# wpeebles/gangealing

Measured on NVIDIA H100. Metric: gangealing_train_images_per_sec_256, higher is better.
Workload: dtype f32

## Files before the change

gangealing_b200/_lib.py:

```python
import ctypes
import os

import torch

_HERE = os.path.dirname(os.path.abspath(__file__))
LIB_PATH = os.path.join(_HERE, "libgg_b200.so")

GG_F32, GG_F16, GG_BF16 = 0, 1, 2
PAD_MODES = {"zeros": 0, "border": 1, "reflection": 2}

_c = ctypes
_P, _I, _L, _F = _c.c_void_p, _c.c_int, _c.c_int64, _c.c_float

SIGNATURES = {
    "gg_version": (_I, []),
    "gg_last_error": (_c.c_char_p, []),
    "gg_sm_count": (_I, []),
    "gg_fused_bias_act": (_I, [_P, _P, _P, _P, _I, _I, _I, _F, _F, _L, _L, _L, _P]),
    "gg_noise_bias_act": (_I, [_P, _P, _P, _P, _P, _P, _I, _F, _F, _L, _L, _L, _P]),
    "gg_channel_scale_workspace": (_L, [_L, _L]),
    "gg_channel_scale": (_I, [_P, _P, _P, _P, _P, _P, _I, _L, _L, _P]),
    "gg_bias_act_backward_workspace": (_L, [_L, _L, _L]),
    "gg_bias_act_backward": (_I, [_P, _P, _P, _P, _P, _I, _F, _F, _L, _L, _L, _P]),
    "gg_upfirdn2d": (_I, [_P, _P, _P, _I, _L] + [_I] * 12 + [_P]),
    "gg_blur_noise_bias_act": (_I, [_P] * 7 + [_I, _L, _L] + [_I] * 9 + [_F, _F, _P]),
    "gg_mipmap_pyramid_elems": (_L, [_L, _I, _I, _I]),
    "gg_mipmap_build": (_I, [_P, _P, _I, _L, _I, _I, _I, _P]),
    "gg_mipmap_build_backward": (_I, [_P, _P, _L, _I, _I, _I, _P]),
    "gg_mipmap_warp_forward": (_I, [_P] * 5 + [_I, _L] + [_I] * 6 + [_F, _F, _I, _P]),
    "gg_warp_sample_indices": (_I, [_P, _P, _L, _I, _I, _I, _I, _F, _F, _I, _P]),
    "gg_stn_sample_forward": (_I, [_P] * 11 + [_I, _I, _L] + [_I] * 9 + [_F, _F, _I, _P]),
    "gg_mipmap_warp_lerp_forward": (_I, [_P] * 5 + [_L, _P, _P, _I, _I, _L] + [_I] * 6 + [_F, _F, _I, _P]),
    "gg_mipmap_warp_lerp_mean": (_I, [_P] * 4 + [_L, _P, _P, _I, _I, _L] + [_I] * 6 + [_F, _F, _I, _I, _P]),
    "gg_track_points_lerp": (_I, [_P] * 6 + [_I, _L, _L, _I, _I, _I, _P]),
    "gg_modconv_wsq": (_I, [_P, _P, _I, _I, _I, _P]),
    "gg_modconv_demod": (_I, [_P, _P, _P, _F, _F, _I, _I, _I, _P]),
    "gg_modconv_demod_batched": (_I, [_I, _P, _P, _P, _P, _P, _P, _F, _I, _P]),
    "gg_modconv_modulate": (_I, [_P, _P, _P, _P, _F, _I, _I, _I, _I, _I, _P]),
    "gg_noise_bias_act_nhwc": (_I, [_P] * 6 + [_I, _F, _F, _L, _I, _L, _P]),
    "gg_nhwc_rowwise_workspace": (_L, [_L, _I, _L]),
    "gg_channel_scale_nhwc": (_I, [_P] * 6 + [_I, _L, _I, _L, _P]),
    "gg_bias_act_backward_nhwc": (_I, [_P] * 5 + [_I, _F, _F, _L, _I, _L, _P]),
    "gg_blur_nhwc_workspace": (_L, [_I, _L] + [_I] * 9),
    "gg_blur_nhwc": (_I, [_P] * 12 + [_I, _L] + [_I] * 12 + [_F, _F, _P]),
    "gg_blur_nhwc_mask": (_I, [_P] * 9 + [_I, _L] + [_I] * 11 + [_F, _F, _P]),
    "gg_styled_tail_nhwc": (_I, [_P] * 12 + [_I, _I, _F, _F, _L, _I, _L, _P]),
    "gg_styled_tail_mask_nhwc": (_I, [_P] * 12 + [_I, _I, _F, _F, _L, _I, _L, _P]),
    "gg_styled_tail_backward_mask_nhwc": (_I, [_P] * 7 + [_I, _F, _F, _L, _I, _L, _P]),
    "gg_styled_tail_backward_workspace": (_L, [_I, _L, _I, _L]),
    "gg_styled_tail_backward_nhwc": (_I, [_P] * 12 + [_I, _F, _F, _L, _I, _L, _L, _P]),
    "gg_tent_downsample_forward": (_I, [_P] * 4 + [_L, _I, _I, _I, _I, _P]),
    "gg_tent_downsample_backward": (_I, [_P] * 4 + [_L, _I, _I, _I, _I, _P]),
    "gg_feature_distance_workspace": (_L, [_L, _I, _L]),
    "gg_feature_distance_forward": (_I, [_P] * 5 + [_I, _L, _I, _L, _F, _P]),
    "gg_feature_distance_backward": (_I, [_P] * 6 + [_I, _L, _I, _L, _F, _P]),
    "gg_bias_relu_pool_nhwc_forward": (_I, [_P, _P, _P, _P, _I, _L, _I, _I, _I, _P]),
    "gg_bias_relu_pool_nhwc_backward": (_I, [_P, _P, _P, _P, _I, _L, _I, _I, _I, _P]),
    "gg_to_rgb_nhwc_workspace": (_L, [_L, _I, _L]),
    "gg_to_rgb_nhwc_forward": (_I, [_P] * 5 + [_L, _I, _L, _P]),
    "gg_to_rgb_nhwc_backward": (_I, [_P] * 6 + [_L, _I, _L, _P]),
    "gg_nn_argmin_workspace": (_L, [_L, _L]),
    "gg_nn_argmin": (_I, [_P, _P, _P, _P, _L, _L, _I, _P]),
    "gg_splat2d_lookup_forward": (_I, [_P] * 8 + [_L, _L, _I, _I, _I, _I, _I, _F, _F, _I, _P]),
    "gg_scale_cast_multi": (_I, [_P, _P, _P, _I, _I, _P]),
    "gg_adam_ema_step": (_I, [_P, _P, _P, _I, _I, _P, _c.c_double, _c.c_double, _c.c_double, _c.c_double, _P]),
    "gg_tv_loss_workspace": (_L, [_L, _I, _I]),
    "gg_tv_loss_forward": (_I, [_P, _P, _P, _L, _I, _I, _P]),
    "gg_tv_loss_backward": (_I, [_P, _P, _P, _L, _I, _I, _P]),
    "gg_splat2d_workspace": (_L, [_L, _I, _I, _I]),
    "gg_splat2d_forward": (_I, [_P] * 6 + [_L, _L, _I, _I, _I, _I, _P]),
    "gg_splat_composite_grid_workspace": (_L, [_L, _L, _I, _I]),
    "gg_splat_composite_grid": (_I, [_P, _P, _L, _P, _P, _P, _P, _F, _F, _L, _L, _L, _I, _I, _I, _I, _I, _I, _P]),
    "gg_splat_lookup_composite_grid": (_I, [_P] * 10 + [_F, _F, _L, _L] + [_I] * 9 + [_P]),
    "gg_flow_compose_forward": (_I, [_P] * 7 + [_L, _I, _I, _I, _P]),
    "gg_flow_compose_backward": (_I, [_P] * 10 + [_L, _I, _I, _I, _P]),
    "gg_mipmap_warp_backward": (_I, [_P] * 7 + [_I, _L] + [_I] * 6 + [_F, _F, _I, _P]),
    "gg_laplacian_blend_workspace": (_L, [_L, _I, _I, _I, _I, _I]),
    "gg_laplacian_blend_forward": (_I, [_P] * 6 + [_L, _I, _I, _I, _I, _I, _P]),
    "gg_laplacian_blend_backward": (_I, [_P] * 9 + [_L, _I, _I, _I, _I, _I, _P]),
    "gg_tv_per_sample": (_I, [_P, _P, _L, _I, _I, _P]),
    "gg_pck_transfer_workspace": (_L, [_L, _L, _I]),
    "gg_pck_transfer": (_I, [_P] * 14 + [_L, _L, _I, _I, _I, _I, _I, _P]),
    "gg_batch_gram": (_I, [_P, _P, _P, _P, _L, _I, _P]),
    "gg_flow_image_grid": (_I, [_P, _P, _P, _L, _I, _I, _I, _I, _P]),
    "gg_image_grid": (_I, [_P, _P, _P, _L, _I, _I, _I, _I, _P]),
    "gg_cluster_accumulate": (_I, [_P] * 5 + [_L, _I, _I, _I, _I, _I] + [_L] * 6 + [_I, _P]),
}

_dll = None
CALLS = 0


def load():
    global _dll
    if _dll is None:
        if not os.path.exists(LIB_PATH):
            raise RuntimeError(
                "libgg_b200.so is missing (%s): build it with `python -m gangealing_b200.build` "
                "(there is no CPU/PyTorch fallback for these ops)" % LIB_PATH)
        dll = ctypes.CDLL(LIB_PATH)
        for name, (res, args) in SIGNATURES.items():
            fn = getattr(dll, name)
            fn.restype = res
            fn.argtypes = args
        _dll = dll
    return _dll


def check(rc, what):
    global CALLS
    CALLS += 1
    if rc != 0:
        msg = load().gg_last_error().decode("utf-8", "replace")
        raise RuntimeError("%s failed (%d): %s" % (what, rc, msg))


def dtype_code(t):
    d = t.dtype
    if d == torch.float32:
        return GG_F32
    if d == torch.float16:
        return GG_F16
    if d == torch.bfloat16:
        return GG_BF16
    raise RuntimeError("gangealing_b200: dtype %s is not supported (float32/float16/bfloat16)" % d)


def require_cuda(*tensors):
    for t in tensors:
        if t is None:
            continue
        if not t.is_cuda:
            raise RuntimeError("gangealing_b200 ops run on CUDA tensors only (got a %s tensor); "
                               "the CPU restatement lives in oracle/ and is test infrastructure" % t.device.type)
        if t.device.index != torch.cuda.current_device():
            raise RuntimeError("gangealing_b200: tensor lives on %s but the current device is cuda:%d; wrap the call in "
                               "`with torch.cuda.device(tensor.device):`" % (t.device, torch.cuda.current_device()))


def ptr(t):
    return None if t is None else t.data_ptr()


def is_nhwc(t):
    return (t.dim() == 4 and t.dtype in (torch.float32, torch.bfloat16) and t.shape[1] > 1 and t.shape[2] * t.shape[3] > 1
            and t.is_contiguous(memory_format=torch.channels_last) and not t.is_contiguous())


def nhwc_vec(t):
    return 8 if t.dtype == torch.bfloat16 else 4


def aligned16(t):
    return t.data_ptr() % 16 == 0


def dense_f32(t):
    if t.dtype != torch.float32 or not t.is_contiguous():
        t = t.float().contiguous()
    return t if aligned16(t) else t.clone()


def tensor_cache(t):
    stamp = (t._version, t.data_ptr(), t.device, t.dtype)
    ent = getattr(t, "_gg_cache", None)
    if ent is None or ent[0] != stamp:
        ent = (stamp, {})
        try:
            t._gg_cache = ent
        except Exception:
            pass
    return ent[1]


def filter_is_separable(kernel):
    memo = tensor_cache(kernel)
    v = memo.get("separable")
    if v is None:
        k = kernel.detach().float().cpu()
        big = k.abs().max()
        if big == 0:
            v = True
        else:
            i0, j0 = divmod(int(k.abs().argmax()), k.shape[1])
            v = bool((k - torch.outer(k[:, j0], k[i0, :]) / k[i0, j0]).abs().max() <= 1e-6 * big)
        memo["separable"] = v
    return v


def flipped_filter(kernel):
    memo = tensor_cache(kernel)
    f = memo.get("flipped")
    if f is None:
        f = torch.flip(kernel.detach(), [0, 1])
        fm = tensor_cache(f)
        fm["flipped"] = kernel.detach()
        if "separable" in memo:
            fm["separable"] = memo["separable"]
        memo["flipped"] = f
    return f


def invalidate(t):
    try:
        t._gg_cache = None
    except Exception:
        pass


def stream():
    return torch.cuda.current_stream().cuda_stream


def sm_count():
    return load().gg_sm_count()


def ship_table(slot, payload):
    capturing = torch.cuda.is_current_stream_capturing()
    ev = slot.get("event")
    if ev is not None and not capturing:
        ev.synchronize()
    slot["host"].copy_(payload)
    slot["dev"].copy_(slot["host"], non_blocking=True)
    if capturing:
        slot["event"] = None
    else:
        ev = torch.cuda.Event()
        ev.record()
        slot["event"] = ev
```

gangealing_b200/csrc/nhwc.cu:

```cuda
#include <cuda.h>

#include "common.cuh"
#include "nhwc_reduce.cuh"

namespace gg {
namespace {

constexpr int kT = 256;

template <typename T>
__global__ void __launch_bounds__(kT)
noise_bias_act_nhwc_kernel(T* __restrict__ out, const T* __restrict__ x, const float* __restrict__ noise,
                           const float* __restrict__ noise_weight, const float* __restrict__ bias,
                           const float* __restrict__ row_scale, float alpha, float gain, int64_t n_vec, int cv,
                           int64_t hw) {
  constexpr int V = ChanVec<T>::V;
  const float nw = noise ? (noise_weight ? __ldg(noise_weight) : 1.f) : 0.f;
  const int64_t base = (static_cast<int64_t>(blockIdx.x) * 4) * kT + threadIdx.x;
  uint4 xv[4];
#pragma unroll
  for (int u = 0; u < 4; ++u) {
    const int64_t v = base + static_cast<int64_t>(u) * kT;
    if (v < n_vec) xv[u] = ldg_stream16(x + v * V);
  }
#pragma unroll
  for (int u = 0; u < 4; ++u) {
    const int64_t v = base + static_cast<int64_t>(u) * kT;
    if (v < n_vec) {
      int64_t pix, n = 0;
      int cq;
      if (n_vec <= 0xffffffffLL) {
        const unsigned v32 = static_cast<unsigned>(v), p32 = v32 / static_cast<unsigned>(cv);
        cq = static_cast<int>(v32 - p32 * static_cast<unsigned>(cv));
        pix = p32;
        if (row_scale) n = p32 / static_cast<unsigned>(hw);
      } else {
        pix = v / cv;
        cq = static_cast<int>(v - pix * cv);
        if (row_scale) n = pix / hw;
      }
      const float nz = noise ? nw * __ldg(noise + pix) : 0.f;
      float xf[V], o[V];
      ChanVec<T>::unpack(xv[u], xf);
#pragma unroll
      for (int q = 0; q < V / 4; ++q) {
        const float4 b = bias ? __ldg(reinterpret_cast<const float4*>(bias) + cq * (V / 4) + q) : make_float4(0.f, 0.f, 0.f, 0.f);
        const float4 r = row_scale ? __ldg(reinterpret_cast<const float4*>(row_scale + n * cv * V) + cq * (V / 4) + q)
                                   : make_float4(1.f, 1.f, 1.f, 1.f);
        const float bb[4] = {b.x, b.y, b.z, b.w}, rr[4] = {r.x, r.y, r.z, r.w};
#pragma unroll
        for (int k = 0; k < 4; ++k) {
          const float t = fmaf(xf[4 * q + k], rr[k], bb[k]) + nz;
          o[4 * q + k] = (t > 0.f ? t : t * alpha) * gain;
        }
      }
      stg_stream16(out + v * V, ChanVec<T>::pack(o));
    }
  }
}

template <typename T, int MODE>
__global__ void __launch_bounds__(kT)
rowwise_nhwc_kernel(T* __restrict__ out, float* __restrict__ partial, const T* __restrict__ x,
                    const T* __restrict__ y, const float* __restrict__ s, float alpha, float gain, int cv,
                    int64_t hw, int chunk, int chunks_per_sample) {
  constexpr int V = ChanVec<T>::V;
  extern __shared__ float red[];
  const int64_t n = blockIdx.x / chunks_per_sample;
  const int ck = blockIdx.x - n * chunks_per_sample;
  const int64_t p0 = static_cast<int64_t>(ck) * chunk, p1 = min(p0 + chunk, hw);
  const int lanes_p = kT / cv > 0 ? kT / cv : 1;
  float acc[V];
#pragma unroll
  for (int k = 0; k < V; ++k) acc[k] = 0.f;
  const int cq = threadIdx.x % cv;
  const int pl = threadIdx.x / cv;
  if (pl < lanes_p) {
    float sv[V];
#pragma unroll
    for (int k = 0; k < V; ++k) sv[k] = (MODE == 0) ? __ldg(s + n * cv * V + cq * V + k) : 1.f;
    const bool has_y = (MODE == 1) || y != nullptr;
    auto body = [&](const uint4 xr, const uint4 yr, int64_t off) {
      float xf[V], yf[V], o[V];
      ChanVec<T>::unpack(xr, xf);
      ChanVec<T>::unpack(yr, yf);
#pragma unroll
      for (int k = 0; k < V; ++k) {
        if (MODE == 0) {
          o[k] = xf[k] * sv[k];
          if (has_y) acc[k] = fmaf(xf[k], yf[k], acc[k]);
        } else {
          o[k] = (yf[k] > 0.f ? xf[k] : xf[k] * alpha) * gain;
          acc[k] += o[k];
        }
      }
      *reinterpret_cast<uint4*>(out + off) = ChanVec<T>::pack(o);
    };
    const uint4 zero = make_uint4(0u, 0u, 0u, 0u);
    int64_t p = p0 + pl;
    for (; p + 3 * lanes_p < p1; p += 4 * lanes_p) {
      uint4 xv[4], yv[4];
      int64_t off[4];
#pragma unroll
      for (int u = 0; u < 4; ++u) {
        off[u] = ((n * hw + p + u * lanes_p) * cv + cq) * V;
        xv[u] = ldg_stream16(x + off[u]);
      }
#pragma unroll
      for (int u = 0; u < 4; ++u) yv[u] = has_y ? ldg_stream16(y + off[u]) : zero;
#pragma unroll
      for (int u = 0; u < 4; ++u) body(xv[u], yv[u], off[u]);
    }
    for (; p < p1; p += lanes_p) {
      const int64_t off = ((n * hw + p) * cv + cq) * V;
      const uint4 xv = ldg_stream16(x + off);
      const uint4 yv = has_y ? ldg_stream16(y + off) : zero;
      body(xv, yv, off);
    }
  }
  if (partial) {
    const int C = cv * V;
    if (pl < lanes_p) {
#pragma unroll
      for (int q = 0; q < V / 4; ++q)
        reinterpret_cast<float4*>(red + pl * C + cq * V)[q] = make_float4(acc[4 * q], acc[4 * q + 1], acc[4 * q + 2], acc[4 * q + 3]);
    }
    __syncthreads();
    for (int c = threadIdx.x; c < C; c += kT) {
      float t = 0.f;
      for (int l = 0; l < lanes_p; ++l) t += red[l * C + c];
      partial[static_cast<int64_t>(blockIdx.x) * C + c] = t;
    }
  }
}

__global__ void __launch_bounds__(kT)
to_rgb_nhwc_fwd_kernel(float* __restrict__ out, const float* __restrict__ x, const float* __restrict__ wm,
                       const float* __restrict__ bias, const float* __restrict__ skip, int c4, int64_t hw, int chunk,
                       int chunks_per_sample) {
  extern __shared__ __align__(16) float wsm[];
  const int64_t n = blockIdx.x / chunks_per_sample;
  const int ck = blockIdx.x - n * chunks_per_sample;
  const int64_t p0 = static_cast<int64_t>(ck) * chunk, p1 = min(p0 + chunk, hw);
  {
    const float4* src = reinterpret_cast<const float4*>(wm + n * 3 * c4 * 4);
    float4* dst = reinterpret_cast<float4*>(wsm);
    for (int i = threadIdx.x; i < 3 * c4; i += kT) dst[i] = __ldg(src + i);
  }
  __syncthreads();
  const float4* w4 = reinterpret_cast<const float4*>(wsm);
  const int l = threadIdx.x & 7, grp = threadIdx.x >> 3;
  const bool vec_ok = (hw & 3) == 0;
  const unsigned gmask = 0xffu << (threadIdx.x & 24);
  for (int64_t pb = p0 + grp * 4; pb < p1; pb += (kT / 8) * 4) {
    float acc[4][3];
#pragma unroll
    for (int u = 0; u < 4; ++u) acc[u][0] = acc[u][1] = acc[u][2] = 0.f;
    const float4* xp[4];
#pragma unroll
    for (int u = 0; u < 4; ++u) {
      const int64_t pu = min(pb + u, p1 - 1);
      xp[u] = reinterpret_cast<const float4*>(x + (n * hw + pu) * c4 * 4);
    }
    for (int q = l; q < c4; q += 8) {
      float4 xv[4];
#pragma unroll
      for (int u = 0; u < 4; ++u) xv[u] = __ldcs(xp[u] + q);
      const float4 w0 = w4[q], w1 = w4[c4 + q], w2 = w4[2 * c4 + q];
#pragma unroll
      for (int u = 0; u < 4; ++u) {
        acc[u][0] = fmaf(xv[u].x, w0.x, fmaf(xv[u].y, w0.y, fmaf(xv[u].z, w0.z, fmaf(xv[u].w, w0.w, acc[u][0]))));
        acc[u][1] = fmaf(xv[u].x, w1.x, fmaf(xv[u].y, w1.y, fmaf(xv[u].z, w1.z, fmaf(xv[u].w, w1.w, acc[u][1]))));
        acc[u][2] = fmaf(xv[u].x, w2.x, fmaf(xv[u].y, w2.y, fmaf(xv[u].z, w2.z, fmaf(xv[u].w, w2.w, acc[u][2]))));
      }
    }
#pragma unroll
    for (int m = 4; m >= 1; m >>= 1)
#pragma unroll
      for (int u = 0; u < 4; ++u)
#pragma unroll
        for (int o = 0; o < 3; ++o) acc[u][o] += __shfl_xor_sync(gmask, acc[u][o], m);
    if (l < 3) {
      const int o = l;
      float r[4];
#pragma unroll
      for (int u = 0; u < 4; ++u) r[u] = (o == 0 ? acc[u][0] : o == 1 ? acc[u][1] : acc[u][2]) + (bias ? __ldg(bias + o) : 0.f);
      const int64_t off = (n * 3 + o) * hw + pb;
      if (vec_ok && pb + 3 < p1) {
        if (skip) {
          const float4 sk = __ldg(reinterpret_cast<const float4*>(skip + off));
          r[0] += sk.x; r[1] += sk.y; r[2] += sk.z; r[3] += sk.w;
        }
        *reinterpret_cast<float4*>(out + off) = make_float4(r[0], r[1], r[2], r[3]);
      } else {
#pragma unroll
        for (int u = 0; u < 4; ++u)
          if (pb + u < p1) out[off + u] = r[u] + (skip ? __ldg(skip + off + u) : 0.f);
      }
    }
  }
}

__global__ void __launch_bounds__(kT)
to_rgb_nhwc_bwd_kernel(float* __restrict__ gx, float* __restrict__ partial, const float* __restrict__ g,
                       const float* __restrict__ x, const float* __restrict__ wm, int c4, int64_t hw, int chunk,
                       int chunks_per_sample) {
  extern __shared__ float red[];
  const int64_t n = blockIdx.x / chunks_per_sample;
  const int ck = blockIdx.x - n * chunks_per_sample;
  const int64_t p0 = static_cast<int64_t>(ck) * chunk, p1 = min(p0 + chunk, hw);
  const int lanes_p = kT / c4 > 0 ? kT / c4 : 1;
  const int cq = threadIdx.x % c4, pl = threadIdx.x / c4;
  float4 a0 = make_float4(0.f, 0.f, 0.f, 0.f), a1 = a0, a2 = a0;
  if (pl < lanes_p) {
    const float4* wp = reinterpret_cast<const float4*>(wm + n * 3 * c4 * 4);
    const float4 w0 = __ldg(wp + cq), w1 = __ldg(wp + c4 + cq), w2 = __ldg(wp + 2 * c4 + cq);
    const float* g0 = g + n * 3 * hw;
    auto body = [&](int64_t p, const float4 xv, float s0, float s1, float s2) {
      float4 o;
      o.x = fmaf(w2.x, s2, fmaf(w1.x, s1, w0.x * s0)); o.y = fmaf(w2.y, s2, fmaf(w1.y, s1, w0.y * s0));
      o.z = fmaf(w2.z, s2, fmaf(w1.z, s1, w0.z * s0)); o.w = fmaf(w2.w, s2, fmaf(w1.w, s1, w0.w * s0));
      if (gx) *reinterpret_cast<float4*>(gx + ((n * hw + p) * c4 + cq) * 4) = o;
      a0.x = fmaf(s0, xv.x, a0.x); a0.y = fmaf(s0, xv.y, a0.y); a0.z = fmaf(s0, xv.z, a0.z); a0.w = fmaf(s0, xv.w, a0.w);
      a1.x = fmaf(s1, xv.x, a1.x); a1.y = fmaf(s1, xv.y, a1.y); a1.z = fmaf(s1, xv.z, a1.z); a1.w = fmaf(s1, xv.w, a1.w);
      a2.x = fmaf(s2, xv.x, a2.x); a2.y = fmaf(s2, xv.y, a2.y); a2.z = fmaf(s2, xv.z, a2.z); a2.w = fmaf(s2, xv.w, a2.w);
    };
    const float4 zero = make_float4(0.f, 0.f, 0.f, 0.f);
    int64_t p = p0 + pl;
    for (; p + 3 * lanes_p < p1; p += 4 * lanes_p) {
      float4 xv[4];
      float s[4][3];
#pragma unroll
      for (int u = 0; u < 4; ++u) {
        const int64_t pu = p + u * lanes_p;
        xv[u] = partial ? __ldcs(reinterpret_cast<const float4*>(x + ((n * hw + pu) * c4 + cq) * 4)) : zero;
        s[u][0] = __ldg(g0 + pu); s[u][1] = __ldg(g0 + hw + pu); s[u][2] = __ldg(g0 + 2 * hw + pu);
      }
#pragma unroll
      for (int u = 0; u < 4; ++u) body(p + u * lanes_p, xv[u], s[u][0], s[u][1], s[u][2]);
    }
    for (; p < p1; p += lanes_p) {
      const float4 xv = partial ? __ldcs(reinterpret_cast<const float4*>(x + ((n * hw + p) * c4 + cq) * 4)) : zero;
      body(p, xv, __ldg(g0 + p), __ldg(g0 + hw + p), __ldg(g0 + 2 * hw + p));
    }
  }
  if (partial) {
    float4* r4 = reinterpret_cast<float4*>(red);
    if (pl < lanes_p) {
      r4[(pl * 3 + 0) * c4 + cq] = a0; r4[(pl * 3 + 1) * c4 + cq] = a1; r4[(pl * 3 + 2) * c4 + cq] = a2;
    }
    __syncthreads();
    for (int i = threadIdx.x; i < 3 * c4; i += kT) {
      float4 t = make_float4(0.f, 0.f, 0.f, 0.f);
      for (int q = 0; q < lanes_p; ++q) {
        const float4 v = r4[q * 3 * c4 + i];
        t.x += v.x; t.y += v.y; t.z += v.z; t.w += v.w;
      }
      reinterpret_cast<float4*>(partial + static_cast<int64_t>(blockIdx.x) * 3 * c4 * 4)[i] = t;
    }
  }
}

template <typename T> struct BlurGeom {
  static constexpr int V = ChanVec<T>::V;
  static constexpr int CB = 8 * V;
  static constexpr int COLS = (V == 4) ? 2 : 1;
  static constexpr int BX = 32 * COLS;
  static constexpr int TW = BX + 3;
  static constexpr int STAGE_ELEMS = 4 * TW * CB;
};
constexpr int kRY = 4;
constexpr int kNS = 3;

struct BlurNhwcParams {
  int n, c, in_h, in_w, out_h, out_w;
  int pad_x0, pad_y0;
  int seg_rows;
  int act;
  float alpha, gain;
};

__device__ __forceinline__ void tma_load_4d(void* smem_dst, const CUtensorMap* tmap, int c0, int x0, int y0, int n0,
                                            uint64_t* bar) {
  asm volatile(
      "cp.async.bulk.tensor.4d.shared::cluster.global.tile.mbarrier::complete_tx::bytes [%0], [%1, {%2, %3, %4, %5}], [%6];"
      ::"r"(smem_u32(smem_dst)), "l"(tmap), "r"(c0), "r"(x0), "r"(y0), "r"(n0), "r"(smem_u32(bar))
      : "memory");
}

template <typename T, int MODE, bool SEP, bool FAST = false>
__global__ void __launch_bounds__(kT, 2)
blur_nhwc_kernel(T* __restrict__ out, T* __restrict__ out2, const __grid_constant__ CUtensorMap tmap,
                 const float* __restrict__ filt, int kh, int kw, const float* __restrict__ noise,
                 const float* __restrict__ noise_weight, const float* __restrict__ bias,
                 const float* __restrict__ row_scale, const float* __restrict__ scale2, const T* __restrict__ mul,
                 float* __restrict__ partial, BlurNhwcParams p) {
  using G = BlurGeom<T>;
  constexpr int V = G::V, CB = G::CB, COLS = G::COLS, BX = G::BX, TW = G::TW;
  constexpr bool FUSED = MODE == 1 || MODE == 3;
  constexpr bool MASK = MODE == 3;
  extern __shared__ __align__(128) unsigned char tiles_raw[];
  T* tiles = reinterpret_cast<T*>(tiles_raw);
  __shared__ uint64_t full_bar[kNS];
  const int tid = threadIdx.x;
  const int cq = tid & 7;
  const int xg = tid >> 3;
  const int chunks = p.c / CB;
  const int bx = blockIdx.x / chunks, cc = blockIdx.x - bx * chunks;
  const int n = blockIdx.z;
  const int oy0 = blockIdx.y * p.seg_rows;
  const int rows_out = min(p.seg_rows, p.out_h - oy0);
  const int x_out0 = bx * BX;
  const int c0 = cc * CB;
  const int iy0 = oy0 - p.pad_y0, ix0 = x_out0 - p.pad_x0;
  const int rows_in = rows_out + 3;
  const int n_stage_iters = (rows_in + kRY - 1) / kRY;
  constexpr uint32_t kStageBytes = G::STAGE_ELEMS * sizeof(T);

  if (tid == 0) {
#pragma unroll
    for (int s = 0; s < kNS; ++s) mbar_init(&full_bar[s], 1);
    mbar_fence_init();
  }
  __syncthreads();
  if (tid == 0) {
#pragma unroll
    for (int s = 0; s < kNS - 1; ++s)
      if (s < n_stage_iters) {
        mbar_expect_tx(&full_bar[s], kStageBytes);
        tma_load_4d(tiles + s * G::STAGE_ELEMS, &tmap, c0, ix0, iy0 + s * kRY, n, &full_bar[s]);
      }
  }

  float kf[4][4];
#pragma unroll
  for (int a = 0; a < 4; ++a)
#pragma unroll
    for (int b = 0; b < 4; ++b)
      kf[a][b] = (a < kh && b < kw) ? __ldg(filt + (kh - 1 - a) * kw + (kw - 1 - b)) : 0.f;
  float ku[4], kv[4];
  {
    int a0 = 0, b0 = 0;
    float big = 0.f;
#pragma unroll
    for (int a = 0; a < 4; ++a)
#pragma unroll
      for (int b = 0; b < 4; ++b)
        if (fabsf(kf[a][b]) > big) { big = fabsf(kf[a][b]); a0 = a; b0 = b; }
    float piv = 1.f;
#pragma unroll
    for (int a = 0; a < 4; ++a)
#pragma unroll
      for (int b = 0; b < 4; ++b)
        if (a == a0 && b == b0) piv = kf[a][b];
    const float inv = big > 0.f ? 1.f / piv : 0.f;
#pragma unroll
    for (int a = 0; a < 4; ++a) {
      float col = 0.f;
#pragma unroll
      for (int b = 0; b < 4; ++b) if (b == b0) col = kf[a][b];
      ku[a] = col * inv;
    }
#pragma unroll
    for (int b = 0; b < 4; ++b) {
      float row = 0.f;
#pragma unroll
      for (int a = 0; a < 4; ++a) if (a == a0) row = kf[a][b];
      kv[b] = row;
    }
  }

  float bq[V], rq[V], sq[V], dacc[V];
#pragma unroll
  for (int k = 0; k < V; ++k) { bq[k] = 0.f; rq[k] = 1.f; sq[k] = 1.f; dacc[k] = 0.f; }
  float nw = 0.f;
  const int64_t nc0 = static_cast<int64_t>(n) * p.c + c0 + cq * V;
  if (MODE != 0) {
    if (row_scale) {
#pragma unroll
      for (int k = 0; k < V; ++k) rq[k] = __ldg(row_scale + nc0 + k);
    }
  }
  if (FUSED) {
    if (bias) {
#pragma unroll
      for (int k = 0; k < V; ++k) bq[k] = __ldg(bias + c0 + cq * V + k);
    }
    if (scale2) {
#pragma unroll
      for (int k = 0; k < V; ++k) sq[k] = __ldg(scale2 + nc0 + k);
    }
    nw = noise ? (noise_weight ? __ldg(noise_weight) : 1.f) : 0.f;
  }
  constexpr bool fast = FUSED && FAST;
  const float neg = (p.act == 3) ? p.alpha : 1.f;
  if (fast) {
#pragma unroll
    for (int k = 0; k < V; ++k) { rq[k] *= p.gain; bq[k] *= p.gain; }
    nw *= p.gain;
  }
  const int xo = x_out0 + COLS * xg;
  const int64_t row_stride = static_cast<int64_t>(p.out_w) * p.c;
  const int64_t obase = ((static_cast<int64_t>(n) * p.out_h + oy0) * p.out_w + xo) * p.c + c0 + cq * V;
  int64_t ocur = obase - 3 * row_stride;
  bool okc[COLS];
#pragma unroll
  for (int j = 0; j < COLS; ++j) okc[j] = xo + j < p.out_w;
  float nzn[kRY][COLS];
#pragma unroll
  for (int rr = 0; rr < kRY; ++rr)
#pragma unroll
    for (int j = 0; j < COLS; ++j) nzn[rr][j] = 0.f;
  const float* noise_base = noise ? noise + (static_cast<int64_t>(n) * p.out_h + oy0) * p.out_w + xo : nullptr;
  auto fetch_noise = [&](int it_) {
#pragma unroll
    for (int rr = 0; rr < kRY; ++rr) {
      const int ro = it_ * kRY + rr - 3;
#pragma unroll
      for (int j = 0; j < COLS; ++j) nzn[rr][j] = 0.f;
      if (ro >= 0 && ro < rows_out) {
        const float* np_ = noise_base + static_cast<int64_t>(ro) * p.out_w;
#pragma unroll
        for (int j = 0; j < COLS; ++j)
          if (okc[j]) nzn[rr][j] = __ldg(np_ + j);
      }
    }
  };
  if (FUSED && noise) fetch_noise(0);

  uint4 mcur[COLS], mnext[COLS];
#pragma unroll
  for (int j = 0; j < COLS; ++j) mcur[j] = mnext[j] = make_uint4(0u, 0u, 0u, 0u);
  auto fetch_mul = [&](int ro_) {
    if (ro_ >= 0 && ro_ < rows_out) {
      const int64_t mo = obase + ro_ * row_stride;
#pragma unroll
      for (int j = 0; j < COLS; ++j)
        if (okc[j]) mnext[j] = __ldg(reinterpret_cast<const uint4*>(mul + mo + static_cast<int64_t>(j) * p.c));
    }
  };
  if (MODE == 2 && mul) { fetch_mul(-3 + 3); }

  float hwin[SEP ? 4 : 1][COLS][V];
  float rwin[SEP ? 1 : 4][COLS + 3][V];
  int r_in = 0;
  for (int it = 0; it < n_stage_iters; ++it) {
    const int stage = it % kNS;
    if (tid == 0) {
      const int nxt = it + kNS - 1;
      if (nxt < n_stage_iters) {
        const int ns = nxt % kNS;
        asm volatile("fence.proxy.async.shared::cta;" ::: "memory");
        mbar_expect_tx(&full_bar[ns], kStageBytes);
        tma_load_4d(tiles + ns * G::STAGE_ELEMS, &tmap, c0, ix0, iy0 + nxt * kRY, n, &full_bar[ns]);
      }
    }
    float nzc[kRY][COLS];
#pragma unroll
    for (int rr = 0; rr < kRY; ++rr)
#pragma unroll
      for (int j = 0; j < COLS; ++j) nzc[rr][j] = nzn[rr][j];
    if (FUSED && noise && it + 1 < n_stage_iters) fetch_noise(it + 1);
    if (MODE == 2 && mul && it + 1 < n_stage_iters) {
#pragma unroll
      for (int rr = 0; rr < kRY; ++rr) {
        const int ro = (it + 1) * kRY + rr - 3;
        if (ro >= 0 && ro < rows_out) {
          const T* mp = mul + obase + ro * row_stride;
#pragma unroll
          for (int j = 0; j < COLS; ++j)
            if (okc[j]) asm volatile("prefetch.global.L2 [%0];" ::"l"(mp + static_cast<int64_t>(j) * p.c));
        }
      }
    }
    mbar_wait(&full_bar[stage], static_cast<uint32_t>((it / kNS) & 1));
    const T* st = tiles + stage * G::STAGE_ELEMS;
#pragma unroll
    for (int rr = 0; rr < kRY; ++rr, ++r_in, ocur += row_stride) {
      if (MODE == 2 && mul) {
#pragma unroll
        for (int j = 0; j < COLS; ++j) mcur[j] = mnext[j];
        fetch_mul(r_in - 3 + 1);
      }
      const uint4* rowp = reinterpret_cast<const uint4*>(st + (rr * TW + COLS * xg) * CB) + cq;
      float q[COLS + 3][V];
#pragma unroll
      for (int i = 0; i < COLS + 3; ++i) ChanVec<T>::unpack(rowp[i * 8], q[i]);
      if constexpr (SEP) {
#pragma unroll
        for (int j = 0; j < COLS; ++j)
#pragma unroll
          for (int k = 0; k < V; ++k) {
            float h = __fmul_rn(kv[0], q[j][k]);
            h = __fmaf_rn(kv[1], q[j + 1][k], h);
            h = __fmaf_rn(kv[2], q[j + 2][k], h);
            h = __fmaf_rn(kv[3], q[j + 3][k], h);
            hwin[rr][j][k] = h;
          }
      } else {
#pragma unroll
        for (int i = 0; i < COLS + 3; ++i)
#pragma unroll
          for (int k = 0; k < V; ++k) rwin[rr][i][k] = q[i][k];
      }
      const int ro = r_in - 3;
      if (ro >= 0 && ro < rows_out) {
#pragma unroll
        for (int j = 0; j < COLS; ++j) {
          float a4[V];
          if constexpr (SEP) {
#pragma unroll
            for (int k = 0; k < V; ++k) {
              float a = __fmul_rn(ku[0], hwin[(rr + 1) & 3][j][k]);
              a = __fmaf_rn(ku[1], hwin[(rr + 2) & 3][j][k], a);
              a = __fmaf_rn(ku[2], hwin[(rr + 3) & 3][j][k], a);
              a = __fmaf_rn(ku[3], hwin[rr][j][k], a);
              a4[k] = a;
            }
          } else {
#pragma unroll
            for (int k = 0; k < V; ++k) a4[k] = 0.f;
#pragma unroll
            for (int a = 0; a < 4; ++a)
#pragma unroll
              for (int b = 0; b < 4; ++b)
#pragma unroll
                for (int k = 0; k < V; ++k) a4[k] = fmaf(kf[a][b], rwin[(rr + 1 + a) & 3][j + b][k], a4[k]);
          }
          const int64_t ooff = ocur + j * p.c;
          if (FUSED) {
            const float nzj = nw * nzc[rr][j];
            float o2[V];
#pragma unroll
            for (int k = 0; k < V; ++k) {
              float t = __fmaf_rn(a4[k], rq[k], __fadd_rn(bq[k], nzj));
              const float tn = __fmul_rn(t, neg);
              if (fast) t = fmaxf(t, tn);
              else t = (t > 0.f ? t : tn) * p.gain;
              a4[k] = t;
              o2[k] = __fmul_rn(t, sq[k]);
            }
            uint32_t word = 0u;
            if (MASK) word = sign_word<V>(sign_bits<T>(a4), cq, 0xffffffffu);
            if (okc[j]) {
              if (MASK) {
                if ((cq * V & 31) == 0) reinterpret_cast<uint32_t*>(out)[ooff >> 5] = word;
              } else if (out) {
                *reinterpret_cast<uint4*>(out + ooff) = ChanVec<T>::pack(a4);
              }
              if (out2) *reinterpret_cast<uint4*>(out2 + ooff) = ChanVec<T>::pack(o2);
            }
          } else if (MODE == 2) {
            if (okc[j]) {
              if (mul) {
                float mf[V];
                ChanVec<T>::unpack(mcur[j], mf);
#pragma unroll
                for (int k = 0; k < V; ++k) dacc[k] = fmaf(a4[k], mf[k], dacc[k]);
              }
#pragma unroll
              for (int k = 0; k < V; ++k) a4[k] *= rq[k];
              *reinterpret_cast<uint4*>(out + ooff) = ChanVec<T>::pack(a4);
            }
          } else {
            if (okc[j]) *reinterpret_cast<uint4*>(out + ooff) = ChanVec<T>::pack(a4);
          }
        }
      }
    }
    __syncthreads();
  }
  if (MODE == 2 && partial) {
    float* red = reinterpret_cast<float*>(tiles_raw);
#pragma unroll
    for (int k = 0; k < V; ++k) red[xg * CB + cq * V + k] = dacc[k];
    __syncthreads();
    if (tid < CB) {
      float t = 0.f;
#pragma unroll 8
      for (int g = 0; g < 32; ++g) t += red[g * CB + tid];
      const int64_t K = static_cast<int64_t>(gridDim.x / chunks) * gridDim.y;
      const int64_t kidx = static_cast<int64_t>(bx) * gridDim.y + blockIdx.y;
      partial[(static_cast<int64_t>(n) * K + kidx) * p.c + c0 + tid] = t;
    }
  }
}

typedef CUresult (*EncodeTiledFn)(CUtensorMap*, CUtensorMapDataType, cuuint32_t, void*, const cuuint64_t*, const cuuint64_t*,
                                  const cuuint32_t*, const cuuint32_t*, CUtensorMapInterleave, CUtensorMapSwizzle,
                                  CUtensorMapL2promotion, CUtensorMapFloatOOBfill);

inline EncodeTiledFn encode_fn() {
  static EncodeTiledFn fn = nullptr;
  if (!fn) {
    void* p = nullptr;
    cudaDriverEntryPointQueryResult q;
    if (cudaGetDriverEntryPoint("cuTensorMapEncodeTiled", &p, cudaEnableDefault, &q) == cudaSuccess &&
        q == cudaDriverEntryPointSuccess)
      fn = reinterpret_cast<EncodeTiledFn>(p);
  }
  return fn;
}

inline int grid1(int64_t total, int per_cta) {
  int64_t g = (total + per_cta - 1) / per_cta;
  return static_cast<int>(g > 0 ? g : 1);
}

}
}

using namespace gg;

extern "C" {

static inline int vec_of(int dtype) { return dtype == GG_BF16 ? 8 : 4; }

int gg_noise_bias_act_nhwc(void* out, const void* x, const float* noise, const float* noise_weight, const float* bias,
                           const float* row_scale, int dtype, float alpha, float scale, int64_t N, int C, int64_t HW,
                           void* stream) {
  if (N < 0 || C < 0 || HW < 0) return fail(GG_ERR_BAD_ARG, "noise_bias_act_nhwc: negative size");
  if (dtype != GG_F32 && dtype != GG_BF16) return fail(GG_ERR_UNSUPPORTED, "noise_bias_act_nhwc: dtype %d not supported", dtype);
  const int64_t numel = N * HW * C;
  if (numel == 0) return GG_OK;
  const int V = vec_of(dtype);
  if (C % V != 0) return fail(GG_ERR_UNSUPPORTED, "noise_bias_act_nhwc: C must be a multiple of %d", V);
  if (!out || !x) return fail(GG_ERR_BAD_ARG, "noise_bias_act_nhwc: null tensor");
  if (!aligned16(bias) || !aligned16(row_scale))
    return fail(GG_ERR_BAD_ARG, "noise_bias_act_nhwc: bias and row_scale must be 16-byte aligned");
  const int64_t n_vec = numel / V;
  const int64_t grid = (n_vec + 4 * kT - 1) / (4 * kT);
  if (grid > 0x7fffffffLL) return fail(GG_ERR_BAD_ARG, "noise_bias_act_nhwc: tensor too large");
  GG_DISPATCH_T(dtype, "noise_bias_act_nhwc",
                (noise_bias_act_nhwc_kernel<T_><<<static_cast<unsigned>(grid), kT, 0, static_cast<cudaStream_t>(stream)>>>(
                    static_cast<T_*>(out), static_cast<const T_*>(x), noise, noise_weight, bias, row_scale, alpha, scale,
                    n_vec, C / V, HW)));
  GG_CHECK_LAUNCH("noise_bias_act_nhwc launch");
  return GG_OK;
}

static int64_t rowwise_chunk(int64_t N, int cv, int64_t HW) {
  const int lanes_p = kT / cv > 0 ? kT / cv : 1;
  const int64_t target = 8LL * sm_count();
  int64_t k = (target + N - 1) / N;
  const int64_t kmax = (HW + 4 * lanes_p - 1) / (4 * lanes_p);
  if (k > kmax) k = kmax;
  if (k < 1) k = 1;
  return (HW + k - 1) / k;
}

int64_t gg_nhwc_rowwise_workspace(int64_t N, int C, int64_t HW) {
  if (N <= 0 || C <= 0 || HW <= 0 || C % 4 != 0) return 0;
  const int64_t chunk = rowwise_chunk(N, C / 4, HW);
  const int64_t chunk8 = (C % 8 == 0) ? rowwise_chunk(N, C / 8, HW) : chunk;
  const int64_t k = (HW + (chunk < chunk8 ? chunk : chunk8) - 1) / (chunk < chunk8 ? chunk : chunk8);
  return N * k * C * static_cast<int64_t>(sizeof(float));
}

static int launch_rowwise(int mode, void* out, float* dst, void* workspace, const void* x, const void* y, const float* s,
                          int dtype, float alpha, float gain, int64_t N, int C, int64_t HW, bool per_sample, void* stream) {
  if (N < 0 || C < 0 || HW < 0) return fail(GG_ERR_BAD_ARG, "nhwc rowwise: negative size");
  if (dtype != GG_F32 && dtype != GG_BF16) return fail(GG_ERR_UNSUPPORTED, "nhwc rowwise: dtype %d not supported", dtype);
  if (N * HW * C == 0) {
    const int64_t sums = (per_sample ? N : 1) * C;
    if (dst && sums > 0) {
      cudaError_t e = cudaMemsetAsync(dst, 0, sums * sizeof(float), static_cast<cudaStream_t>(stream));
      if (e != cudaSuccess) return cuda_fail(e, "nhwc rowwise memset");
    }
    return GG_OK;
  }
  const int V = vec_of(dtype);
  if (C % V != 0 || C / V > kT) return fail(GG_ERR_UNSUPPORTED, "nhwc rowwise: C must be a multiple of %d and <= %d", V, V * kT);
  if (!out || !x) return fail(GG_ERR_BAD_ARG, "nhwc rowwise: null tensor");
  if (dst && !workspace) return fail(GG_ERR_BAD_ARG, "nhwc rowwise: reduction needs a workspace");
  const int cv = C / V;
  const int64_t chunk64 = rowwise_chunk(N, cv, HW);
  if (chunk64 > 0x7fffffffLL) return fail(GG_ERR_BAD_ARG, "nhwc rowwise: plane too large");
  const int chunk = static_cast<int>(chunk64);
  const int K = static_cast<int>((HW + chunk - 1) / chunk);
  const int64_t grid = N * K;
  if (grid > 0x7fffffffLL) return fail(GG_ERR_BAD_ARG, "nhwc rowwise: too many CTAs");
  const int lanes_p = kT / cv > 0 ? kT / cv : 1;
  const size_t smem = static_cast<size_t>(lanes_p) * C * sizeof(float);
  float* partial = dst ? static_cast<float*>(workspace) : nullptr;
  auto st = static_cast<cudaStream_t>(stream);
  const unsigned g = static_cast<unsigned>(grid);
  if (mode == 0) {
    GG_DISPATCH_T(dtype, "nhwc rowwise",
                  (rowwise_nhwc_kernel<T_, 0><<<g, kT, smem, st>>>(static_cast<T_*>(out), partial, static_cast<const T_*>(x),
                                                                 dst ? static_cast<const T_*>(y) : nullptr, s, alpha, gain,
                                                                 cv, HW, chunk, K)));
  } else {
    GG_DISPATCH_T(dtype, "nhwc rowwise",
                  (rowwise_nhwc_kernel<T_, 1><<<g, kT, smem, st>>>(static_cast<T_*>(out), partial, static_cast<const T_*>(x),
                                                                 static_cast<const T_*>(y), s, alpha, gain, cv, HW, chunk, K)));
  }
  GG_CHECK_LAUNCH("nhwc rowwise launch");
  if (dst) {
    const int64_t rows = per_sample ? N : 1;
    const int kk = per_sample ? K : static_cast<int>(N * K);
    nhwc_finish_kernel<<<static_cast<unsigned>(rows * ((C + 31) / 32)), dim3(32, 32), 0, st>>>(dst, partial, rows, kk, C);
    GG_CHECK_LAUNCH("nhwc finish launch");
  }
  return GG_OK;
}

int gg_channel_scale_nhwc(void* out, float* row_dot, void* workspace, const void* x, const void* y, const float* s,
                          int dtype, int64_t N, int C, int64_t HW, void* stream) {
  if (!s) return fail(GG_ERR_BAD_ARG, "channel_scale_nhwc: null scale");
  if (row_dot && !y) return fail(GG_ERR_BAD_ARG, "channel_scale_nhwc: row_dot needs y");
  return launch_rowwise(0, out, row_dot, workspace, x, y, s, dtype, 0.f, 1.f, N, C, HW, true, stream);
}

int gg_bias_act_backward_nhwc(void* gx, float* grad_bias, void* workspace, const void* g, const void* out_saved,
                              int dtype, float alpha, float scale, int64_t N, int C, int64_t HW, void* stream) {
  if (!out_saved) return fail(GG_ERR_BAD_ARG, "bias_act_backward_nhwc: null saved output");
  return launch_rowwise(1, gx, grad_bias, workspace, g, out_saved, nullptr, dtype, alpha, scale, N, C, HW, false, stream);
}

int64_t gg_to_rgb_nhwc_workspace(int64_t N, int C, int64_t HW) { return 3 * gg_nhwc_rowwise_workspace(N, C, HW); }

int gg_to_rgb_nhwc_forward(float* out, const float* x, const float* wm, const float* bias, const float* skip, int64_t N,
                           int C, int64_t HW, void* stream) {
  if (N < 0 || C < 0 || HW < 0) return fail(GG_ERR_BAD_ARG, "to_rgb_nhwc: negative size");
  if (N * HW == 0) return GG_OK;
  if (C < 32 || C % 32 != 0 || C > 1024) return fail(GG_ERR_UNSUPPORTED, "to_rgb_nhwc: C must be a multiple of 32, <= 1024");
  if (!out || !x || !wm) return fail(GG_ERR_BAD_ARG, "to_rgb_nhwc: null tensor");
  if (!aligned16(wm) || (HW % 4 == 0 && (!aligned16(skip) || !aligned16(out))))
    return fail(GG_ERR_BAD_ARG, "to_rgb_nhwc: wm (and skip, out when HW %% 4 == 0) must be 16-byte aligned");
  const int64_t target = 8LL * sm_count();
  int64_t k = (target + N - 1) / N;
  const int64_t kmax = (HW + 127) / 128;
  if (k > kmax) k = kmax;
  if (k < 1) k = 1;
  int64_t chunk = ((HW + k - 1) / k + 127) / 128 * 128;
  if (chunk > 0x7fffff00LL) return fail(GG_ERR_BAD_ARG, "to_rgb_nhwc: plane too large");
  const int K = static_cast<int>((HW + chunk - 1) / chunk);
  const int64_t grid = N * K;
  if (grid > 0x7fffffffLL) return fail(GG_ERR_BAD_ARG, "to_rgb_nhwc: too many CTAs");
  to_rgb_nhwc_fwd_kernel<<<static_cast<unsigned>(grid), kT, static_cast<size_t>(3) * C * sizeof(float),
                           static_cast<cudaStream_t>(stream)>>>(out, x, wm, bias, skip, C / 4, HW, static_cast<int>(chunk), K);
  GG_CHECK_LAUNCH("to_rgb_nhwc forward launch");
  return GG_OK;
}

int gg_to_rgb_nhwc_backward(float* gx, float* gwm, void* workspace, const float* g, const float* x, const float* wm,
                            int64_t N, int C, int64_t HW, void* stream) {
  if (N < 0 || C < 0 || HW < 0) return fail(GG_ERR_BAD_ARG, "to_rgb_nhwc backward: negative size");
  if (N * HW == 0 || C == 0) {
    if (gwm && N * C > 0) {
      cudaError_t e = cudaMemsetAsync(gwm, 0, N * 3 * C * sizeof(float), static_cast<cudaStream_t>(stream));
      if (e != cudaSuccess) return cuda_fail(e, "to_rgb_nhwc backward memset");
    }
    return GG_OK;
  }
  if (C % 4 != 0 || C > 1024) return fail(GG_ERR_UNSUPPORTED, "to_rgb_nhwc backward: C must be a multiple of 4, <= 1024");
  if (!g || !wm || (!gx && !gwm)) return fail(GG_ERR_BAD_ARG, "to_rgb_nhwc backward: null tensor");
  if (gwm && (!x || !workspace)) return fail(GG_ERR_BAD_ARG, "to_rgb_nhwc backward: gwm needs x and a workspace");
  if (!aligned16(wm)) return fail(GG_ERR_BAD_ARG, "to_rgb_nhwc backward: wm must be 16-byte aligned");
  const int c4 = C / 4;
  const int64_t chunk64 = rowwise_chunk(N, c4, HW);
  if (chunk64 > 0x7fffffffLL) return fail(GG_ERR_BAD_ARG, "to_rgb_nhwc backward: plane too large");
  const int chunk = static_cast<int>(chunk64);
  const int K = static_cast<int>((HW + chunk - 1) / chunk);
  const int64_t grid = N * K;
  if (grid > 0x7fffffffLL) return fail(GG_ERR_BAD_ARG, "to_rgb_nhwc backward: too many CTAs");
  const int lanes_p = kT / c4 > 0 ? kT / c4 : 1;
  const size_t smem = static_cast<size_t>(lanes_p) * 3 * C * sizeof(float);
  auto st = static_cast<cudaStream_t>(stream);
  float* partial = gwm ? static_cast<float*>(workspace) : nullptr;
  to_rgb_nhwc_bwd_kernel<<<static_cast<unsigned>(grid), kT, smem, st>>>(gx, partial, g, x, wm, c4, HW, chunk, K);
  GG_CHECK_LAUNCH("to_rgb_nhwc backward launch");
  if (gwm) {
    nhwc_finish_kernel<<<static_cast<unsigned>(N * ((3 * C + 31) / 32)), dim3(32, 32), 0, st>>>(gwm, partial, N, K, 3 * C);
    GG_CHECK_LAUNCH("to_rgb_nhwc finish launch");
  }
  return GG_OK;
}

struct BlurPlan {
  int out_h, out_w, xblocks, chunks, segs, seg_rows;
};
static int blur_plan(BlurPlan* pl, int dtype, int64_t N, int C, int in_h, int in_w, int kernel_h, int kernel_w, int pad_x0,
                     int pad_x1, int pad_y0, int pad_y1) {
  const int V = vec_of(dtype);
  const int CB = 8 * V, BX = (V == 4) ? 64 : 32;
  if (C % CB != 0) return fail(GG_ERR_UNSUPPORTED, "blur_nhwc: C must be a multiple of %d", CB);
  pl->out_h = in_h + pad_y0 + pad_y1 - kernel_h + 1;
  pl->out_w = in_w + pad_x0 + pad_x1 - kernel_w + 1;
  if (pl->out_h < 1 || pl->out_w < 1) return fail(GG_ERR_BAD_ARG, "blur_nhwc: empty output");
  pl->xblocks = (pl->out_w + BX - 1) / BX;
  pl->chunks = C / CB;
  const int64_t base_ctas = static_cast<int64_t>(pl->xblocks) * pl->chunks * (N > 0 ? N : 1);
  int segs = static_cast<int>((2LL * 2 * sm_count() + base_ctas - 1) / base_ctas);
  int seg_rows = (pl->out_h + segs - 1) / segs;
  if (seg_rows < 16) seg_rows = pl->out_h < 16 ? pl->out_h : 16;
  seg_rows = (seg_rows + 3) / 4 * 4;
  pl->seg_rows = seg_rows;
  pl->segs = (pl->out_h + seg_rows - 1) / seg_rows;
  return GG_OK;
}

int64_t gg_blur_nhwc_workspace(int dtype, int64_t N, int C, int in_h, int in_w, int kernel_h, int kernel_w, int pad_x0,
                               int pad_x1, int pad_y0, int pad_y1) {
  BlurPlan pl;
  if (N <= 0 || C <= 0 || (dtype != GG_F32 && dtype != GG_BF16)) return 0;
  if (blur_plan(&pl, dtype, N, C, in_h, in_w, kernel_h, kernel_w, pad_x0, pad_x1, pad_y0, pad_y1) != GG_OK) return 0;
  return N * static_cast<int64_t>(pl.xblocks) * pl.segs * C * static_cast<int64_t>(sizeof(float));
}

}

template <typename T>
static int launch_blur(void* out, void* out2, const void* in, const float* kernel, const float* noise,
                       const float* noise_weight, const float* bias, const float* row_scale, const float* scale2,
                       const void* mul, float* row_dot, void* workspace, int64_t N, int C, int in_h, int in_w, int kernel_h,
                       int kernel_w, int separable, int pad_x0, int pad_x1, int pad_y0, int pad_y1, int mode, int act,
                       float alpha, float scale, void* stream, int dtype, bool out_is_mask) {
  using G = BlurGeom<T>;
  BlurPlan pl;
  int rc = blur_plan(&pl, dtype, N, C, in_h, in_w, kernel_h, kernel_w, pad_x0, pad_x1, pad_y0, pad_y1);
  if (rc != GG_OK) return rc;
  EncodeTiledFn enc = encode_fn();
  if (!enc) return fail(GG_ERR_CUDA, "blur_nhwc: cuTensorMapEncodeTiled is not available from this driver");
  struct MapKey { const void* ptr; int64_t n; int c, h, w, es; };
  struct MapEnt { MapKey key; CUtensorMap map; bool valid; };
  static thread_local MapEnt cache[16] = {};
  static thread_local unsigned cache_next = 0;
  const MapKey key = {in, N, C, in_h, in_w, static_cast<int>(sizeof(T))};
  const CUtensorMap* cached = nullptr;
  for (int i = 0; i < 16 && !cached; ++i)
    if (cache[i].valid && cache[i].key.ptr == key.ptr && cache[i].key.n == key.n && cache[i].key.c == key.c &&
        cache[i].key.h == key.h && cache[i].key.w == key.w && cache[i].key.es == key.es)
      cached = &cache[i].map;
  CUtensorMap tmap;
  if (cached) tmap = *cached;
  const cuuint64_t es = sizeof(T);
  const cuuint64_t gdim[4] = {static_cast<cuuint64_t>(C), static_cast<cuuint64_t>(in_w), static_cast<cuuint64_t>(in_h),
                              static_cast<cuuint64_t>(N)};
  const cuuint64_t gstr[3] = {static_cast<cuuint64_t>(C) * es, static_cast<cuuint64_t>(in_w) * C * es,
                              static_cast<cuuint64_t>(in_h) * in_w * C * es};
  const cuuint32_t box[4] = {G::CB, G::TW, kRY, 1};
  const cuuint32_t estr[4] = {1, 1, 1, 1};
  if (!cached) {
    const CUresult r = enc(&tmap, sizeof(T) == 4 ? CU_TENSOR_MAP_DATA_TYPE_FLOAT32 : CU_TENSOR_MAP_DATA_TYPE_BFLOAT16, 4,
                           const_cast<void*>(in), gdim, gstr, box, estr, CU_TENSOR_MAP_INTERLEAVE_NONE,
                           CU_TENSOR_MAP_SWIZZLE_NONE, CU_TENSOR_MAP_L2_PROMOTION_L2_128B, CU_TENSOR_MAP_FLOAT_OOB_FILL_NONE);
    if (r != CUDA_SUCCESS) return fail(GG_ERR_CUDA, "blur_nhwc: cuTensorMapEncodeTiled failed (%d)", static_cast<int>(r));
    MapEnt& e = cache[cache_next++ % 16];
    e.key = key; e.map = tmap; e.valid = true;
  }
  BlurNhwcParams p;
  p.n = static_cast<int>(N); p.c = C; p.in_h = in_h; p.in_w = in_w; p.out_h = pl.out_h; p.out_w = pl.out_w;
  p.pad_x0 = pad_x0; p.pad_y0 = pad_y0;
  p.act = act; p.alpha = alpha; p.gain = scale;
  p.seg_rows = pl.seg_rows;
  const dim3 grid(static_cast<unsigned>(pl.xblocks * pl.chunks), static_cast<unsigned>(pl.segs), static_cast<unsigned>(N));
  const size_t smem = static_cast<size_t>(kNS) * G::STAGE_ELEMS * sizeof(T);
  static DeviceOnce configured;
  if (configured.needed()) {
    cudaError_t e = cudaSuccess;
    const void* kernels[12] = {reinterpret_cast<const void*>(blur_nhwc_kernel<T, 0, true>),
                              reinterpret_cast<const void*>(blur_nhwc_kernel<T, 0, false>),
                              reinterpret_cast<const void*>(blur_nhwc_kernel<T, 1, true, false>),
                              reinterpret_cast<const void*>(blur_nhwc_kernel<T, 1, false, false>),
                              reinterpret_cast<const void*>(blur_nhwc_kernel<T, 1, true, true>),
                              reinterpret_cast<const void*>(blur_nhwc_kernel<T, 1, false, true>),
                              reinterpret_cast<const void*>(blur_nhwc_kernel<T, 3, true, false>),
                              reinterpret_cast<const void*>(blur_nhwc_kernel<T, 3, false, false>),
                              reinterpret_cast<const void*>(blur_nhwc_kernel<T, 3, true, true>),
                              reinterpret_cast<const void*>(blur_nhwc_kernel<T, 3, false, true>),
                              reinterpret_cast<const void*>(blur_nhwc_kernel<T, 2, true>),
                              reinterpret_cast<const void*>(blur_nhwc_kernel<T, 2, false>)};
    for (int i = 0; i < 12 && e == cudaSuccess; ++i)
      e = cudaFuncSetAttribute(kernels[i], cudaFuncAttributeMaxDynamicSharedMemorySize, static_cast<int>(smem));
    if (e != cudaSuccess) return cuda_fail(e, "blur_nhwc smem opt-in");
    configured.done();
  }
  auto st = static_cast<cudaStream_t>(stream);
  float* partial = (mode == 2 && row_dot) ? static_cast<float*>(workspace) : nullptr;
  const bool fast = scale > 0.f && ((act == 3 && alpha >= 0.f && alpha <= 1.f) || act == 1);
#define GG_BLUR(M_, S_, F_)                                                                                          \
  blur_nhwc_kernel<T, M_, S_, F_><<<grid, kT, smem, st>>>(static_cast<T*>(out), static_cast<T*>(out2), tmap, kernel, kernel_h, \
                                                         kernel_w, noise, noise_weight, bias, row_scale, scale2,     \
                                                         static_cast<const T*>(mul), partial, p)
  if (mode == 1 && out_is_mask) {
    if (fast) { if (separable) GG_BLUR(3, true, true); else GG_BLUR(3, false, true); }
    else { if (separable) GG_BLUR(3, true, false); else GG_BLUR(3, false, false); }
  }
  else if (mode == 1) {
    if (fast) { if (separable) GG_BLUR(1, true, true); else GG_BLUR(1, false, true); }
    else { if (separable) GG_BLUR(1, true, false); else GG_BLUR(1, false, false); }
  }
  else if (mode == 2) { if (separable) GG_BLUR(2, true, false); else GG_BLUR(2, false, false); }
  else { if (separable) GG_BLUR(0, true, false); else GG_BLUR(0, false, false); }
#undef GG_BLUR
  GG_CHECK_LAUNCH("blur_nhwc launch");
  if (partial) {
    const int K = pl.xblocks * pl.segs;
    nhwc_finish_kernel<<<static_cast<unsigned>(N * ((C + 31) / 32)), dim3(32, 32), 0, st>>>(row_dot, partial, N, K, C);
    GG_CHECK_LAUNCH("blur_nhwc finish launch");
  }
  return GG_OK;
}

extern "C" {

int gg_blur_nhwc(void* out, void* out2, const void* in, const float* kernel, const float* noise, const float* noise_weight,
                 const float* bias, const float* row_scale, const float* scale2, const void* mul, float* row_dot,
                 void* workspace, int dtype, int64_t N, int C, int in_h, int in_w, int kernel_h, int kernel_w, int separable,
                 int pad_x0, int pad_x1, int pad_y0, int pad_y1, int mode, int act, float alpha, float scale, void* stream) {
  if (N < 0 || C < 0 || in_h < 1 || in_w < 1) return fail(GG_ERR_BAD_ARG, "blur_nhwc: bad shape");
  if (kernel_h < 1 || kernel_w < 1 || kernel_h > 4 || kernel_w > 4) return fail(GG_ERR_UNSUPPORTED, "blur_nhwc: filter must be <= 4x4");
  if (mode < 0 || mode > 2) return fail(GG_ERR_BAD_ARG, "blur_nhwc: mode must be 0 (blur), 1 (fused tail) or 2 (adjoint epilogue)");
  if (act != 1 && act != 3) return fail(GG_ERR_UNSUPPORTED, "blur_nhwc: act must be 1 or 3");
  if (dtype != GG_F32 && dtype != GG_BF16) return fail(GG_ERR_UNSUPPORTED, "blur_nhwc: dtype %d not supported (fp32 or bf16)", dtype);
  if (N == 0 || C == 0) return GG_OK;
  if (!in || !kernel) return fail(GG_ERR_BAD_ARG, "blur_nhwc: null tensor");
  if (mode == 1 ? (!out && !out2) : !out) return fail(GG_ERR_BAD_ARG, "blur_nhwc: null output");
  if (mode != 1 && out2) return fail(GG_ERR_BAD_ARG, "blur_nhwc: out2 belongs to the fused tail (mode 1)");
  if (mode == 2 && row_dot && (!mul || !workspace)) return fail(GG_ERR_BAD_ARG, "blur_nhwc: row_dot needs `mul` and a workspace");
  if (N > 65535) return fail(GG_ERR_UNSUPPORTED, "blur_nhwc: batch > 65535");
  if (mode == 0) { noise = nullptr; noise_weight = nullptr; bias = nullptr; row_scale = nullptr; scale2 = nullptr; }
  GG_DISPATCH_T(dtype, "blur_nhwc",
                return launch_blur<T_>(out, out2, in, kernel, noise, noise_weight, bias, row_scale, scale2, mul, row_dot,
                                       workspace, N, C, in_h, in_w, kernel_h, kernel_w, separable, pad_x0, pad_x1, pad_y0,
                                       pad_y1, mode, act, alpha, scale, stream, dtype, false));
  return GG_OK;
}

int gg_blur_nhwc_mask(void* mask, void* out2, const void* in, const float* kernel, const float* noise,
                      const float* noise_weight, const float* bias, const float* row_scale, const float* scale2, int dtype,
                      int64_t N, int C, int in_h, int in_w, int kernel_h, int kernel_w, int separable, int pad_x0, int pad_x1,
                      int pad_y0, int pad_y1, int act, float alpha, float scale, void* stream) {
  if (N < 0 || C < 0 || in_h < 1 || in_w < 1) return fail(GG_ERR_BAD_ARG, "blur_nhwc_mask: bad shape");
  if (kernel_h < 1 || kernel_w < 1 || kernel_h > 4 || kernel_w > 4) return fail(GG_ERR_UNSUPPORTED, "blur_nhwc_mask: filter must be <= 4x4");
  if (act != 1 && act != 3) return fail(GG_ERR_UNSUPPORTED, "blur_nhwc_mask: act must be 1 or 3");
  if (dtype != GG_F32 && dtype != GG_BF16) return fail(GG_ERR_UNSUPPORTED, "blur_nhwc_mask: dtype %d not supported (fp32 or bf16)", dtype);
  if (N == 0 || C == 0) return GG_OK;
  if (!in || !kernel) return fail(GG_ERR_BAD_ARG, "blur_nhwc_mask: null tensor");
  if (!mask) return fail(GG_ERR_BAD_ARG, "blur_nhwc_mask: null mask");
  if (out2 && !scale2) return fail(GG_ERR_BAD_ARG, "blur_nhwc_mask: out2 needs scale2");
  if (N > 65535) return fail(GG_ERR_UNSUPPORTED, "blur_nhwc_mask: batch > 65535");
  GG_DISPATCH_T(dtype, "blur_nhwc_mask",
                return launch_blur<T_>(mask, out2, in, kernel, noise, noise_weight, bias, row_scale, scale2, nullptr, nullptr,
                                       nullptr, N, C, in_h, in_w, kernel_h, kernel_w, separable, pad_x0, pad_x1, pad_y0,
                                       pad_y1, 1, act, alpha, scale, stream, dtype, true));
  return GG_OK;
}

}
```

gangealing_b200/op/fused_act.py:

```python
import torch
from torch import nn
from torch.autograd import Function

from .. import _lib
from . import nhwc


def fused_bias_act_raw(x, bias, ref, act, grad, alpha, scale):
    _lib.require_cuda(x, bias, ref)
    cl = _lib.is_nhwc(x) and (ref is None or (ref.shape == x.shape and ref.stride() == x.stride()))
    if not cl:
        x = x.contiguous()
    if bias is not None and bias.numel() == 0:
        bias = None
    if ref is not None and ref.numel() == 0:
        ref = None
    if bias is not None:
        bias = bias.to(x.dtype).contiguous()
    if ref is not None:
        if ref.shape != x.shape or ref.dtype != x.dtype:
            raise RuntimeError("fused_bias_act: ref must match the input's shape and dtype")
        if not cl:
            ref = ref.contiguous()
    step_b = 1
    if not cl:
        for s in x.shape[2:]:
            step_b *= s
    out = torch.empty_like(x)
    rc = _lib.load().gg_fused_bias_act(out.data_ptr(), x.data_ptr(), _lib.ptr(bias), _lib.ptr(ref),
                                       _lib.dtype_code(x), act, grad, alpha, scale, x.numel(), step_b,
                                       0 if bias is None else bias.numel(), _lib.stream())
    _lib.check(rc, "gg_fused_bias_act")
    return out


def bias_act_backward_raw(grad_output, out, alpha, scale, want_bias_grad):
    _lib.require_cuda(grad_output, out)
    if nhwc.rowwise_ok(out) and grad_output.shape == out.shape:
        g = grad_output.contiguous(memory_format=torch.channels_last)
        if g.dtype != out.dtype:
            g = g.to(out.dtype)
        return nhwc.bias_act_backward(g, out, alpha, scale, want_bias_grad)
    g = grad_output.contiguous()
    out = out.contiguous()
    if g.shape != out.shape or g.dtype != out.dtype:
        raise RuntimeError("bias_act_backward: grad_output/out mismatch")
    n = g.shape[0] if g.dim() > 0 else 1
    c = g.shape[1] if g.dim() > 1 else 1
    hw = 1
    for s in g.shape[2:]:
        hw *= s
    gx = torch.empty_like(g)
    lib = _lib.load()
    grad_bias = ws = None
    if want_bias_grad:
        grad_bias = torch.empty(c, dtype=torch.float32, device=g.device)
        ws = torch.empty(max(1, lib.gg_bias_act_backward_workspace(n, c, hw) // 4), dtype=torch.float32,
                         device=g.device)
    rc = lib.gg_bias_act_backward(gx.data_ptr(), _lib.ptr(grad_bias), _lib.ptr(ws), g.data_ptr(), out.data_ptr(),
                                  _lib.dtype_code(g), alpha, scale, n, c, hw, _lib.stream())
    _lib.check(rc, "gg_bias_act_backward")
    return gx, grad_bias


class _FusedLeakyReLUGrad(Function):
    @staticmethod
    def forward(ctx, grad_output, out, negative_slope, scale, want_bias_grad, bias_dtype=None):
        gx, grad_bias = bias_act_backward_raw(grad_output, out, negative_slope, scale, want_bias_grad)
        ctx.save_for_backward(out)
        ctx.cfg = (negative_slope, scale)
        if grad_bias is None:
            grad_bias = gx.new_zeros(())
        else:
            grad_bias = grad_bias.to(bias_dtype if bias_dtype is not None else gx.dtype)
        return gx, grad_bias

    @staticmethod
    def backward(ctx, gradgrad_input, gradgrad_bias):
        (out,) = ctx.saved_tensors
        negative_slope, scale = ctx.cfg
        bias = gradgrad_bias if (gradgrad_bias is not None and gradgrad_bias.dim() == 1) else None
        gradgrad_out = fused_bias_act_raw(gradgrad_input, bias, out, 3, 1, negative_slope, scale)
        return gradgrad_out, None, None, None, None, None


class FusedLeakyReLUFunction(Function):
    @staticmethod
    def forward(ctx, input, bias, negative_slope, scale):
        _lib.require_cuda(input, bias)
        if nhwc.elementwise_ok(input) and (bias is None or bias.numel() in (0, input.shape[1])):
            b = bias if (bias is not None and bias.numel() > 0) else None
            out = nhwc.noise_bias_act(input, None, None, b, None, negative_slope, scale)
        else:
            out = fused_bias_act_raw(input, bias, None, 3, 0, negative_slope, scale)
        ctx.save_for_backward(out)
        ctx.cfg = (negative_slope, scale, bias.dtype if bias is not None else None)
        return out

    @staticmethod
    def backward(ctx, grad_output):
        (out,) = ctx.saved_tensors
        negative_slope, scale, bias_dtype = ctx.cfg
        want_bias = ctx.needs_input_grad[1]
        grad_input, grad_bias = _FusedLeakyReLUGrad.apply(grad_output, out, negative_slope, scale, want_bias, bias_dtype)
        return grad_input, (grad_bias if want_bias else None), None, None


def fused_leaky_relu(input, bias, negative_slope=0.2, scale=2 ** 0.5):
    return FusedLeakyReLUFunction.apply(input, bias, negative_slope, scale)


class FusedLeakyReLU(nn.Module):

    def __init__(self, channel, negative_slope=0.2, scale=2 ** 0.5):
        super().__init__()
        self.bias = nn.Parameter(torch.zeros(channel))
        self.negative_slope = negative_slope
        self.scale = scale

    def forward(self, input):
        return fused_leaky_relu(input, self.bias.type(input.dtype), self.negative_slope, self.scale)
```

gangealing_b200/op/nhwc.py:

```python
import torch

from .. import _lib

CL = torch.channels_last

TIMING = None


def elementwise_ok(t):
    return _lib.is_nhwc(t) and t.shape[1] % _lib.nhwc_vec(t) == 0 and _lib.aligned16(t)


def rowwise_ok(t):
    return elementwise_ok(t) and t.shape[1] // _lib.nhwc_vec(t) <= 256


def blur_ok(t, kh, kw, up=(1, 1), down=(1, 1)):
    return (_lib.is_nhwc(t) and t.shape[1] % (8 * _lib.nhwc_vec(t)) == 0 and kh <= 4 and kw <= 4
            and up == (1, 1) and down == (1, 1) and _lib.aligned16(t))


def _f32(t, numel=None):
    if t is None:
        return None
    t = _lib.dense_f32(t.detach())
    if numel is not None and t.numel() != numel:
        raise RuntimeError("channels-last op: expected %d fp32 values, got %d" % (numel, t.numel()))
    return t


def noise_plane(noise, n, h, w):
    if noise is None:
        return None
    noise = noise.detach()
    if noise.numel() != n * h * w:
        noise = noise.expand(n, 1, h, w)
    return noise.float().contiguous()


def sign_mask_empty(n, c, h, w, device):
    if c % 32:
        raise RuntimeError("sign mask: C = %d is not a multiple of 32" % c)
    return torch.empty((n, h, w, c // 32), dtype=torch.int32, device=device)


def blur(x, kernel, pad, mode=0, noise=None, noise_weight=None, bias=None, row_scale=None, scale2=None, want_out=True,
         want_out2=False, mul=None, want_dot=False, negative_slope=0.2, gain=1.0, act=3, want_mask=False):
    n, c, in_h, in_w = x.shape
    taps = kernel.detach()
    if taps.dtype != torch.float32 or not taps.is_contiguous():
        taps = taps.float().contiguous()
    kh, kw = taps.shape
    out_h = in_h + pad[2] + pad[3] - kh + 1
    out_w = in_w + pad[0] + pad[1] - kw + 1
    if out_h < 1 or out_w < 1:
        raise RuntimeError("blur: empty output (%d x %d)" % (out_h, out_w))
    lib = _lib.load()
    code = _lib.dtype_code(x)

    def empty():
        return torch.empty((n, c, out_h, out_w), dtype=x.dtype, device=x.device, memory_format=CL)
    if want_mask and mode != 1:
        raise RuntimeError("blur: the sign mask belongs to the fused tail (mode 1)")
    if want_mask:
        out = sign_mask_empty(n, c, out_h, out_w, x.device)
    else:
        out = empty() if (want_out or mode != 1) else None
    out2 = empty() if (mode == 1 and want_out2) else None
    nz = noise_plane(noise, n, out_h, out_w) if mode == 1 else None
    dot = ws = None
    if mode == 2 and want_dot:
        if (mul is None or mul.shape != (n, c, out_h, out_w) or mul.dtype != x.dtype or not mul.is_contiguous(memory_format=CL)
                or not _lib.aligned16(mul)):
            raise RuntimeError("blur (adjoint epilogue): `mul` must be a 16-byte-aligned channels-last tensor of the output's "
                               "shape and dtype")
        dot = torch.empty((n, c), dtype=torch.float32, device=x.device)
        nbytes = lib.gg_blur_nhwc_workspace(code, n, c, in_h, in_w, kh, kw, pad[0], pad[1], pad[2], pad[3])
        ws = torch.empty(max(1, nbytes // 4), dtype=torch.float32, device=x.device)
    timed = TIMING is not None and mode == 1
    if timed:
        ev0, ev1 = torch.cuda.Event(enable_timing=True), torch.cuda.Event(enable_timing=True)
        ev0.record()
    nw, b, rs, s2 = _f32(noise_weight, 1), _f32(bias, c), _f32(row_scale, n * c), _f32(scale2, n * c)
    sep = 1 if _lib.filter_is_separable(kernel) else 0
    if want_mask:
        rc = lib.gg_blur_nhwc_mask(out.data_ptr(), _lib.ptr(out2), x.data_ptr(), taps.data_ptr(), _lib.ptr(nz), _lib.ptr(nw),
                                   _lib.ptr(b), _lib.ptr(rs), _lib.ptr(s2), code, n, c, in_h, in_w, kh, kw, sep, pad[0],
                                   pad[1], pad[2], pad[3], act, negative_slope, gain, _lib.stream())
    else:
        rc = lib.gg_blur_nhwc(_lib.ptr(out), _lib.ptr(out2), x.data_ptr(), taps.data_ptr(), _lib.ptr(nz),
                              _lib.ptr(nw), _lib.ptr(b), _lib.ptr(rs),
                              _lib.ptr(s2), _lib.ptr(mul if dot is not None else None), _lib.ptr(dot), _lib.ptr(ws),
                              code, n, c, in_h, in_w, kh, kw, sep, pad[0], pad[1],
                              pad[2], pad[3], mode, act, negative_slope, gain, _lib.stream())
    _lib.check(rc, "gg_blur_nhwc_mask" if want_mask else "gg_blur_nhwc")
    if timed:
        ev1.record()
        es = x.element_size()
        writes = (out is not None and not want_mask) + (out2 is not None)
        TIMING.append((ev0, ev1, es * n * c * (in_h * in_w + writes * out_h * out_w) + (4 * n * out_h * out_w if nz is not None else 0)
                       + (out.numel() * 4 if want_mask else 0)
                       + 4 * ((2 + (scale2 is not None)) * c + 1 + kh * kw)))
    return out, out2, dot


def noise_bias_act(x, noise, noise_weight, bias, row_scale, negative_slope, gain):
    n, c, h, w = x.shape
    out = torch.empty_like(x)
    nz, nw, b, rs = noise_plane(noise, n, h, w), _f32(noise_weight, 1), _f32(bias, c), _f32(row_scale, n * c)
    rc = _lib.load().gg_noise_bias_act_nhwc(out.data_ptr(), x.data_ptr(), _lib.ptr(nz), _lib.ptr(nw), _lib.ptr(b),
                                            _lib.ptr(rs), _lib.dtype_code(x), negative_slope, gain, n, c, h * w,
                                            _lib.stream())
    _lib.check(rc, "gg_noise_bias_act_nhwc")
    return out


def bias_act_backward(g, out_saved, negative_slope, gain, want_bias_grad):
    n, c, h, w = out_saved.shape
    lib = _lib.load()
    gx = torch.empty_like(out_saved)
    grad_bias = ws = None
    if want_bias_grad:
        grad_bias = torch.empty(c, dtype=torch.float32, device=g.device)
        ws = torch.empty(max(1, lib.gg_nhwc_rowwise_workspace(n, c, h * w) // 4), dtype=torch.float32, device=g.device)
    rc = lib.gg_bias_act_backward_nhwc(gx.data_ptr(), _lib.ptr(grad_bias), _lib.ptr(ws), g.data_ptr(), out_saved.data_ptr(),
                                       _lib.dtype_code(out_saved), negative_slope, gain, n, c, h * w, _lib.stream())
    _lib.check(rc, "gg_bias_act_backward_nhwc")
    return gx, grad_bias


def channel_scale(x, s, y=None):
    n, c, h, w = x.shape
    lib = _lib.load()
    out = torch.empty_like(x)
    dot = ws = None
    if y is not None:
        dot = torch.empty((n, c), dtype=torch.float32, device=x.device)
        ws = torch.empty(max(1, lib.gg_nhwc_rowwise_workspace(n, c, h * w) // 4), dtype=torch.float32, device=x.device)
    sc = _f32(s, n * c)
    rc = lib.gg_channel_scale_nhwc(out.data_ptr(), _lib.ptr(dot), _lib.ptr(ws), x.data_ptr(), _lib.ptr(y), sc.data_ptr(),
                                   _lib.dtype_code(x), n, c, h * w, _lib.stream())
    _lib.check(rc, "gg_channel_scale_nhwc")
    return out, dot


def _activation_like(t, like, who, name):
    if t is not None and (t.shape != like.shape or t.dtype != like.dtype or not t.is_contiguous(memory_format=CL)
                          or not _lib.aligned16(t)):
        raise RuntimeError("%s: %s must be a 16-byte-aligned channels-last tensor of the activation's shape and dtype"
                           % (who, name))


def _rgb_grad_ok(g_rgb, n, h, w, who):
    if g_rgb is not None and (g_rgb.shape != (n, 3, h, w) or g_rgb.dtype != torch.float32 or not g_rgb.is_contiguous()):
        raise RuntimeError("%s: g_rgb must be a dense fp32 (N, 3, H, W) tensor" % who)


def styled_tail(raw, noise, noise_weight, bias, demod, s_next, wm, rgb_bias, skip, want_out, negative_slope, gain, act=3,
                want_mask=False):
    _activation_like(raw, raw, "styled_tail", "raw")
    n, c, h, w = raw.shape
    if want_mask:
        out = sign_mask_empty(n, c, h, w, raw.device)
    else:
        out = torch.empty_like(raw) if want_out else None
    xs = torch.empty_like(raw) if s_next is not None else None
    rgb = torch.empty((n, 3, h, w), dtype=torch.float32, device=raw.device) if wm is not None else None
    sk = None
    if skip is not None and rgb is not None:
        sk = skip.detach()
        if sk.dtype != torch.float32 or not sk.is_contiguous():
            sk = sk.float().contiguous()
        if sk.shape != rgb.shape:
            raise RuntimeError("styled_tail: skip must be (N, 3, H, W)")
    consts = [noise_plane(noise, n, h, w), _f32(noise_weight, 1), _f32(bias, c), _f32(demod, n * c), _f32(s_next, n * c),
              _f32(wm, n * 3 * c), _f32(rgb_bias, 3)]
    lib = _lib.load()
    entry = lib.gg_styled_tail_mask_nhwc if want_mask else lib.gg_styled_tail_nhwc
    rc = entry(_lib.ptr(out), _lib.ptr(xs), _lib.ptr(rgb), raw.data_ptr(), *[_lib.ptr(t) for t in consts], _lib.ptr(sk),
               _lib.dtype_code(raw), act, negative_slope, gain, n, c, h * w, _lib.stream())
    _lib.check(rc, "gg_styled_tail_mask_nhwc" if want_mask else "gg_styled_tail_nhwc")
    return out, xs, rgb


def styled_tail_backward(g_xs, g_rgb, out_saved, raw, s_next, demod, wm, want_ds, want_dd, want_dwm, negative_slope, gain):
    n, c, h, w = out_saved.shape
    lib = _lib.load()
    dev = out_saved.device
    want_ds = want_ds and g_xs is not None
    want_dd = want_dd and raw is not None
    want_dwm = want_dwm and g_rgb is not None
    for name, t in (("out_saved", out_saved), ("g_xs", g_xs), ("raw", raw if want_dd else None)):
        _activation_like(t, out_saved, "styled_tail_backward", name)
    _rgb_grad_ok(g_rgb, n, h, w, "styled_tail_backward")
    g_raw = torch.empty_like(out_saved)
    rows = int(want_ds) + int(want_dd) + 3 * int(want_dwm)
    block = torch.empty((n, rows, c), dtype=torch.float32, device=dev) if rows else None
    r = 0
    d_s = d_d = d_w = None
    if want_ds:
        d_s = block[:, r]; r += 1
    if want_dd:
        d_d = block[:, r]; r += 1
    if want_dwm:
        d_w = block[:, r:r + 3]
    code = _lib.dtype_code(out_saved)
    ws = None
    if rows:
        ws = torch.empty(max(1, lib.gg_styled_tail_backward_workspace(code, n, c, h * w) // 4), dtype=torch.float32, device=dev)
    consts = [_f32(s_next, n * c), _f32(demod, n * c), _f32(wm, n * 3 * c)]
    rc = lib.gg_styled_tail_backward_nhwc(g_raw.data_ptr(), _lib.ptr(d_s), _lib.ptr(d_d), _lib.ptr(d_w), _lib.ptr(ws),
                                          _lib.ptr(g_xs), _lib.ptr(g_rgb), out_saved.data_ptr(),
                                          _lib.ptr(raw if want_dd else None),
                                          *[_lib.ptr(t) for t in consts],
                                          code, negative_slope, gain, n, c, h * w, rows * c, _lib.stream())
    _lib.check(rc, "gg_styled_tail_backward_nhwc")
    return g_raw, d_s, d_d, d_w


def styled_tail_backward_mask(g_xs, g_rgb, mask, s_next, demod, wm, negative_slope, gain, dtype):
    n, h, w, words = mask.shape
    c = 32 * words
    g_raw = torch.empty((n, c, h, w), dtype=dtype, device=mask.device, memory_format=CL)
    _activation_like(g_xs, g_raw, "styled_tail_backward_mask", "g_xs")
    _rgb_grad_ok(g_rgb, n, h, w, "styled_tail_backward_mask")
    consts = [_f32(s_next, n * c), _f32(demod, n * c), _f32(wm, n * 3 * c)]
    rc = _lib.load().gg_styled_tail_backward_mask_nhwc(g_raw.data_ptr(), _lib.ptr(g_xs), _lib.ptr(g_rgb), mask.data_ptr(),
                                                       *[_lib.ptr(t) for t in consts], _lib.dtype_code(g_raw),
                                                       negative_slope, gain, n, c, h * w, _lib.stream())
    _lib.check(rc, "gg_styled_tail_backward_mask_nhwc")
    return g_raw
```

gangealing_b200/opset.py:

```python
import types

_cached = None


def cuda_ops():
    global _cached
    if _cached is None:
        from . import op as _op
        from .op import modconv as _mod
        from .stn import flow as _flow
        from .stn import sampling as _smp
        from .splat2d import nn_argmin as _nn_argmin
        from .splat2d import splat2d as _splat2d
        from .splat2d import splat2d_lookup as _splat2d_lookup
        from .splat2d import track_points_lerp as _track_points_lerp
        from .splat2d import splat_composite_grid as _splat_composite_grid
        from .splat2d import splat_lookup_composite_grid as _splat_lookup_composite_grid
        from .splat2d import laplacian_blend as _laplacian_blend
        from .op import feature_distance as _fd
        from .op import vgg_pool as _vp
        from .evaluation import ops as _ev
        from .op import pca as _pca
        from .op import grids as _grids
        _cached = types.SimpleNamespace(
            name="sm_90a",
            upfirdn2d=_op.upfirdn2d,
            fused_leaky_relu=_op.fused_leaky_relu,
            noise_bias_act=_op.noise_bias_act,
            blur_noise_bias_act=_op.blur_noise_bias_act,
            conv2d=_op.conv2d_gradfix.conv2d,
            conv_transpose2d=_op.conv2d_gradfix.conv_transpose2d,
            modulated_weight=_mod.modulated_weight,
            modulated_conv2d=_mod.modulated_conv2d,
            channel_scale=_mod.channel_scale,
            mipmap_warp=_smp.mipmap_warp,
            grid_sample=_smp.grid_sample_bilinear,
            bilinear_downsample=_smp.bilinear_downsample,
            flow_compose=_flow.flow_compose,
            stn_sample_affine=_smp.stn_sample_affine,
            stn_sample_flow=_smp.stn_sample_flow,
            splat2d=_splat2d,
            splat2d_lookup=_splat2d_lookup,
            nn_argmin=_nn_argmin,
            laplacian_blend=_laplacian_blend,
            feature_distance=_fd.feature_distance,
            feature_distance_stacked=_fd.feature_distance_stacked,
            bias_relu_pool=_vp.bias_relu_pool,
            bias_relu_pool_supported=_vp.supported,
            tv_per_sample=_ev.tv_per_sample,
            pck_transfer_points=_ev.pck_transfer_points,
            batch_gram=_pca.batch_gram,
            mipmap_warp_lerp=_smp.mipmap_warp_lerp,
            mipmap_warp_lerp_mean=_smp.mipmap_warp_lerp_mean,
            track_points_lerp=_track_points_lerp,
            splat_composite_grid=_splat_composite_grid,
            splat_lookup_composite_grid=_splat_lookup_composite_grid,
            flow_image_grid=_grids.flow_image_grid,
            image_grid=_grids.image_grid,
            cluster_accumulate=_grids.cluster_accumulate,
        )
    return _cached
```

gangealing_b200/stylegan2/networks.py:

```python
import math
import random

import torch
from torch import nn
from torch.nn import functional as F

from ..opset import cuda_ops


def make_kernel(k):
    k = torch.tensor(k, dtype=torch.float32)
    if k.ndim == 1:
        k = k[None, :] * k[:, None]
    return k / k.sum()


class PixelNorm(nn.Module):
    def forward(self, input):
        return input * torch.rsqrt(torch.mean(input ** 2, dim=1, keepdim=True) + 1e-8)


class _FirModule(nn.Module):

    def __init__(self, kernel, up, down, pad, ops):
        super().__init__()
        self.register_buffer("kernel", kernel)
        self.up, self.down, self.pad = up, down, pad
        self.ops = ops if ops is not None else cuda_ops()

    def forward(self, input):
        return self.ops.upfirdn2d(input, self.kernel, up=self.up, down=self.down, pad=self.pad)


class Upsample(_FirModule):
    def __init__(self, kernel, factor=2, ops=None):
        k = make_kernel(kernel) * (factor ** 2)
        p = k.shape[0] - factor
        super().__init__(k, factor, 1, ((p + 1) // 2 + factor - 1, p // 2), ops)
        self.factor = factor


class Downsample(_FirModule):
    def __init__(self, kernel, factor=2, ops=None):
        k = make_kernel(kernel)
        p = k.shape[0] - factor
        super().__init__(k, 1, factor, ((p + 1) // 2, p // 2), ops)
        self.factor = factor


class Blur(_FirModule):
    def __init__(self, kernel, pad, upsample_factor=1, ops=None):
        k = make_kernel(kernel)
        if upsample_factor > 1:
            k = k * (upsample_factor ** 2)
        super().__init__(k, 1, 1, pad, ops)


class EqualConv2d(nn.Module):
    def __init__(self, in_channel, out_channel, kernel_size, stride=1, padding=0, bias=True, ops=None):
        super().__init__()
        self.weight = nn.Parameter(torch.randn(out_channel, in_channel, kernel_size, kernel_size))
        self.scale = 1 / math.sqrt(in_channel * kernel_size ** 2)
        self.stride, self.padding = stride, padding
        self.bias = nn.Parameter(torch.zeros(out_channel)) if bias else None
        self.ops = ops if ops is not None else cuda_ops()

    scaler = None

    def forward(self, input, gain=1.0):
        w = self.scaler.get(self, input.dtype, gain) if self.scaler is not None and input.is_cuda else None
        if w is None:
            w = self.weight * (self.scale * gain)
        b = self.bias
        if w.dtype != input.dtype:
            w = w.to(input.dtype)
        if b is not None and b.dtype != input.dtype:
            b = b.to(input.dtype)
        return self.ops.conv2d(input, w, bias=b, stride=self.stride, padding=self.padding)

    def __repr__(self):
        return (f"{self.__class__.__name__}({self.weight.shape[1]}, {self.weight.shape[0]},"
                f" {self.weight.shape[2]}, stride={self.stride}, padding={self.padding})")


class EqualLinear(nn.Module):
    def __init__(self, in_dim, out_dim, bias=True, bias_init=0, lr_mul=1, activation=None, ops=None):
        super().__init__()
        self.weight = nn.Parameter(torch.randn(out_dim, in_dim).div_(lr_mul))
        self.bias = nn.Parameter(torch.zeros(out_dim).fill_(bias_init)) if bias else None
        self.activation = activation
        self.scale = (1 / math.sqrt(in_dim)) * lr_mul
        self.lr_mul = lr_mul
        self.ops = ops if ops is not None else cuda_ops()

    scaler = None

    def forward(self, input):
        w = self.scaler.get(self, input.dtype) if self.scaler is not None and input.is_cuda else None
        if w is None:
            w = self.weight * self.scale
        if self.activation:
            out = F.linear(input, w)
            return self.ops.fused_leaky_relu(out, self.bias * self.lr_mul)
        return F.linear(input, w, bias=self.bias * self.lr_mul)

    def __repr__(self):
        return f"{self.__class__.__name__}({self.weight.shape[1]}, {self.weight.shape[0]})"


class ScaledLeakyReLU(nn.Module):
    def __init__(self, negative_slope=0.2):
        super().__init__()
        self.negative_slope = negative_slope

    def forward(self, input):
        return F.leaky_relu(input, negative_slope=self.negative_slope) * math.sqrt(2)


class FusedLeakyReLU(nn.Module):

    def __init__(self, channel, negative_slope=0.2, scale=2 ** 0.5, ops=None):
        super().__init__()
        self.bias = nn.Parameter(torch.zeros(channel))
        self.negative_slope, self.scale = negative_slope, scale
        self.ops = ops if ops is not None else cuda_ops()

    def forward(self, input):
        bias = self.bias if input.dtype == torch.bfloat16 else self.bias.type(input.dtype)
        return self.ops.fused_leaky_relu(input, bias, self.negative_slope, self.scale)


class ModulatedConv2d(nn.Module):

    def __init__(self, in_channel, out_channel, kernel_size, style_dim, demodulate=True, upsample=False,
                 downsample=False, blur_kernel=[1, 3, 3, 1], normalize=False, ops=None):
        super().__init__()
        self.eps = 1e-8
        self.kernel_size, self.in_channel, self.out_channel = kernel_size, in_channel, out_channel
        self.upsample, self.downsample, self.normalize = upsample, downsample, normalize
        self.ops = ops if ops is not None else cuda_ops()
        if upsample:
            factor = 2
            p = (len(blur_kernel) - factor) - (kernel_size - 1)
            self.blur = Blur(blur_kernel, pad=((p + 1) // 2 + factor - 1, p // 2 + 1), upsample_factor=factor, ops=ops)
        if downsample:
            factor = 2
            p = (len(blur_kernel) - factor) + (kernel_size - 1)
            self.blur = Blur(blur_kernel, pad=((p + 1) // 2, p // 2), ops=ops)
        self.scale = 1 / math.sqrt(in_channel * kernel_size ** 2)
        self.padding = kernel_size // 2
        self.weight = nn.Parameter(torch.randn(1, out_channel, in_channel, kernel_size, kernel_size))
        self.modulation = EqualLinear(style_dim, in_channel, bias_init=1, ops=ops)
        self.demodulate = demodulate

    def __repr__(self):
        return (f"{self.__class__.__name__}({self.in_channel}, {self.out_channel}, {self.kernel_size}, "
                f"upsample={self.upsample}, downsample={self.downsample})")

    def conv_raw(self, input, style):
        style = self.modulation(style)
        plain = not (self.normalize or (input.dtype == torch.float16 and self.demodulate)) and not self.downsample
        if plain:
            return self.ops.modulated_conv2d(input, self.weight, style, self.scale, self.demodulate, self.upsample,
                                             self.padding, self.eps)
        return self._reference_formulation(input, style), None

    def forward(self, input, style, fuse_blur=True):
        raw, demod = self.conv_raw(input, style)
        if demod is not None:
            raw = self.ops.channel_scale(raw, demod)
        if self.upsample and fuse_blur:
            return self.blur(raw)
        return raw

    def _reference_formulation(self, input, style):
        batch, in_channel, height, width = input.shape
        weight = self.weight
        scale = self.scale
        if self.normalize or (input.dtype == torch.float16 and self.demodulate):
            style = style / torch.max(torch.abs(style))
            fan = torch.tensor(in_channel * weight.size(3) * weight.size(4), dtype=torch.float32)
            weight = scale * weight * torch.sqrt(1.0 / fan) / torch.amax(torch.abs(scale * weight), dim=(2, 3, 4), keepdims=True)
            scale = 1.0
        w = self.ops.modulated_weight(weight, style, scale, self.demodulate, transposed=self.upsample, eps=self.eps)
        w = w.type(input.dtype)
        x = input.reshape(1, batch * in_channel, height, width)
        if self.upsample:
            out = self.ops.conv_transpose2d(x, w, padding=0, stride=2, groups=batch)
        elif self.downsample:
            xb = self.blur(input)
            out = self.ops.conv2d(xb.reshape(1, batch * in_channel, xb.shape[2], xb.shape[3]), w, padding=0, stride=2,
                                  groups=batch)
        else:
            out = self.ops.conv2d(x, w, padding=self.padding, groups=batch)
        return out.view(batch, self.out_channel, out.shape[2], out.shape[3])


class NoiseInjection(nn.Module):
    def __init__(self):
        super().__init__()
        self.weight = nn.Parameter(torch.zeros(1))

    @staticmethod
    def sample(batch, height, width, like):
        return like.new_empty(batch, 1, height, width).normal_()

    def forward(self, image, noise=None):
        if noise is None:
            noise = self.sample(image.shape[0], image.shape[2], image.shape[3], image)
        return image + self.weight.type(image.dtype) * noise.type(image.dtype)


class ConstantInput(nn.Module):
    def __init__(self, channel, size=4):
        super().__init__()
        self.input = nn.Parameter(torch.randn(1, channel, size, size))
        self.size = size

    def forward(self, input):
        return self.input.repeat(input.shape[0], 1, 1, 1)


class StyledConv(nn.Module):

    def __init__(self, in_channel, out_channel, kernel_size, style_dim, upsample=False, blur_kernel=[1, 3, 3, 1],
                 demodulate=True, normalize=False, ops=None):
        super().__init__()
        self.conv = ModulatedConv2d(in_channel, out_channel, kernel_size, style_dim, upsample=upsample,
                                    blur_kernel=blur_kernel, demodulate=demodulate, normalize=normalize, ops=ops)
        self.noise = NoiseInjection()
        self.activate = FusedLeakyReLU(out_channel, ops=ops)
        self.ops = ops if ops is not None else cuda_ops()

    def forward(self, input, style, noise=None):
        act = self.activate
        raw, demod = self.conv.conv_raw(input, style)
        if self.conv.upsample:
            blur = self.conv.blur
            out_h = raw.shape[2] + blur.pad[0] + blur.pad[1] - blur.kernel.shape[0] + 1
            out_w = raw.shape[3] + blur.pad[0] + blur.pad[1] - blur.kernel.shape[1] + 1
            if noise is None:
                noise = NoiseInjection.sample(raw.shape[0], out_h, out_w, raw)
            return self.ops.blur_noise_bias_act(raw, blur.kernel, blur.pad, noise, self.noise.weight, act.bias,
                                                act.negative_slope, act.scale, row_scale=demod)
        if noise is None:
            noise = NoiseInjection.sample(raw.shape[0], raw.shape[2], raw.shape[3], raw)
        return self.ops.noise_bias_act(raw, noise, self.noise.weight, act.bias, act.negative_slope, act.scale,
                                       row_scale=demod)


class ToRGB(nn.Module):
    def __init__(self, in_channel, style_dim, upsample=True, blur_kernel=[1, 3, 3, 1], normalize=False, ops=None):
        super().__init__()
        if upsample:
            self.upsample = Upsample(blur_kernel, ops=ops)
        self.conv = ModulatedConv2d(in_channel, 3, 1, style_dim, demodulate=False, normalize=normalize, ops=ops)
        self.bias = nn.Parameter(torch.zeros(1, 3, 1, 1))

    def forward(self, input, style, skip=None):
        conv = self.conv
        up = self.upsample(skip) if skip is not None else None
        if not (conv.normalize or conv.downsample or conv.upsample or conv.demodulate):
            out, _ = conv.ops.modulated_conv2d(input, conv.weight, conv.modulation(style), conv.scale, False, False,
                                               conv.padding, conv.eps, bias=self.bias, skip=up)
            return out
        out = conv(input, style) + self.bias.type(input.dtype)
        if up is not None:
            out = out.float() + up
        return out


class ConvLayer(nn.Sequential):

    def __init__(self, in_channel, out_channel, kernel_size, downsample=False, blur_kernel=[1, 3, 3, 1], bias=True,
                 activate=True, ops=None):
        layers = []
        if downsample:
            factor = 2
            p = (len(blur_kernel) - factor) + (kernel_size - 1)
            layers.append(Blur(blur_kernel, pad=((p + 1) // 2, p // 2), ops=ops))
            stride, self.padding = 2, 0
        else:
            stride, self.padding = 1, kernel_size // 2
        layers.append(EqualConv2d(in_channel, out_channel, kernel_size, padding=self.padding, stride=stride,
                                  bias=bias and not activate, ops=ops))
        if activate:
            layers.append(FusedLeakyReLU(out_channel, ops=ops) if bias else ScaledLeakyReLU(0.2))
        super().__init__(*layers)


class ResBlock(nn.Module):
    def __init__(self, in_channel, out_channel, blur_kernel=[1, 3, 3, 1], downsample=True, ops=None):
        super().__init__()
        self.conv1 = ConvLayer(in_channel, in_channel, 3, ops=ops)
        self.conv2 = ConvLayer(in_channel, out_channel, 3, downsample=downsample, ops=ops)
        self.skip = ConvLayer(in_channel, out_channel, 1, downsample=downsample, activate=False, bias=False, ops=ops)

    def forward(self, input):
        act, skip_conv = self.conv2[-1], self.skip[-1]
        if (input.is_cuda and isinstance(act, FusedLeakyReLU) and getattr(act.ops, "name", None) == "sm_90a"
                and isinstance(skip_conv, EqualConv2d) and skip_conv.bias is None):
            inv = 1.0 / math.sqrt(2)
            main = self.conv1(input)
            for layer in list(self.conv2)[:-1]:
                main = layer(main)
            bias = act.bias if main.dtype == torch.bfloat16 else act.bias.type(main.dtype)
            main = act.ops.fused_leaky_relu(main, bias, act.negative_slope, act.scale * inv)
            side = input
            for layer in list(self.skip)[:-1]:
                side = layer(side)
            return main + skip_conv(side, gain=inv)
        return (self.conv2(self.conv1(input)) + self.skip(input)) / math.sqrt(2)


def channel_table(channel_multiplier):
    return {4: 512, 8: 512, 16: 512, 32: 512, 64: 256 * channel_multiplier, 128: 128 * channel_multiplier,
            256: 64 * channel_multiplier, 512: 32 * channel_multiplier, 1024: 16 * channel_multiplier}


class Generator(nn.Module):

    def __init__(self, size, style_dim, n_mlp, channel_multiplier=2, blur_kernel=[1, 3, 3, 1], lr_mlp=0.01,
                 num_fp16_res=0, run_fp32=True, ops=None):
        super().__init__()
        self.size, self.style_dim = size, style_dim
        self.style = nn.Sequential(PixelNorm(), *[EqualLinear(style_dim, style_dim, lr_mul=lr_mlp, activation="fused_lrelu", ops=ops)
                                                  for _ in range(n_mlp)])
        self.channels = channel_table(channel_multiplier)
        self.input = ConstantInput(self.channels[4])
        self.conv1 = StyledConv(self.channels[4], self.channels[4], 3, style_dim, blur_kernel=blur_kernel, ops=ops)
        self.to_rgb1 = ToRGB(self.channels[4], style_dim, upsample=False, ops=ops)
        self.log_size = int(math.log(size, 2))
        self.num_layers = (self.log_size - 2) * 2 + 1
        self.convs, self.upsamples, self.to_rgbs = nn.ModuleList(), nn.ModuleList(), nn.ModuleList()
        self.noises = nn.Module()
        for layer_idx in range(self.num_layers):
            res = (layer_idx + 5) // 2
            self.noises.register_buffer(f"noise_{layer_idx}", torch.randn(1, 1, 2 ** res, 2 ** res))
        in_channel = self.channels[4]
        for i in range(3, self.log_size + 1):
            mixed = i > self.log_size - num_fp16_res
            out_channel = self.channels[2 ** i]
            self.convs.append(StyledConv(in_channel, out_channel, 3, style_dim, upsample=True, blur_kernel=blur_kernel,
                                         normalize=mixed, ops=ops))
            self.convs.append(StyledConv(out_channel, out_channel, 3, style_dim, blur_kernel=blur_kernel,
                                         normalize=mixed, ops=ops))
            self.to_rgbs.append(ToRGB(out_channel, style_dim, normalize=False, ops=ops))
            in_channel = out_channel
        self.n_latent = self.log_size * 2 - 2
        self.num_fp16_res, self.run_fp32 = num_fp16_res, run_fp32
        self.channels_last = False
        self.act_dtype = torch.float32
        self.fuse_synthesis = True

    def ops_are_native(self):
        return getattr(self.conv1.ops, "name", None) == "sm_90a"

    def make_noise(self, batch_size=1):
        device = self.input.input.device
        noises = [torch.randn(batch_size, 1, 4, 4, device=device)]
        for i in range(3, self.log_size + 1):
            noises += [torch.randn(batch_size, 1, 2 ** i, 2 ** i, device=device) for _ in range(2)]
        return noises

    def batch_latent(self, n_latent):
        return self.style(torch.randn(n_latent, self.style_dim, device=self.input.input.device))

    def mean_latent(self, n_latent):
        return self.batch_latent(n_latent).mean(dim=0, keepdim=True)

    def get_latent(self, input):
        return self.style(input)

    def forward(self, styles, mapping_only=False, return_latents=False, inject_index=None, truncation=1,
                truncation_latent=None, input_is_latent=False, noise=None, randomize_noise=True):
        if not input_is_latent:
            styles = [self.style(s) for s in styles]
            if mapping_only:
                return styles
        if noise is None:
            noise = [None] * self.num_layers if randomize_noise else \
                [getattr(self.noises, f"noise_{i}") for i in range(self.num_layers)]
        if truncation < 1:
            styles = [truncation_latent + truncation * (styles[0] - truncation_latent), styles[0]]
        row_needs_grad = None
        if len(styles) < 2 or inject_index == self.n_latent:
            inject_index = self.n_latent
            latent = styles[0].unsqueeze(1).repeat(1, inject_index, 1) if styles[0].ndim < 3 else styles[0]
        else:
            if inject_index is None:
                inject_index = random.randint(1, self.n_latent - 1)
            latent = torch.cat([styles[0].unsqueeze(1).repeat(1, inject_index, 1),
                                styles[1].unsqueeze(1).repeat(1, self.n_latent - inject_index, 1)], 1)
            row_needs_grad = [styles[0].requires_grad] * inject_index + [styles[1].requires_grad] * (self.n_latent - inject_index)

        if self.channels_last and self.fuse_synthesis and self.ops_are_native():
            from ..op import styled_fused
            if styled_fused.fusable(self, latent, self.act_dtype):
                image = styled_fused.synthesis(self, latent, noise, self.act_dtype, row_needs_grad)
                return (image, latent) if return_latents else (image, None)
        x0 = self.input(latent)
        if self.channels_last:
            x0 = x0.contiguous(memory_format=torch.channels_last)
        out = self.conv1(x0, latent[:, 0], noise=noise[0])
        skip = self.to_rgb1(out, latent[:, 1])
        i = 1
        for j, (up, conv, n_up, n_conv, to_rgb) in enumerate(
                zip(self.convs[::2], self.convs[1::2], noise[1::2], noise[2::2], self.to_rgbs), 3):
            half = j > self.log_size - self.num_fp16_res and not self.run_fp32
            out = out.type(torch.float16 if half else torch.float32)
            out = up(out, latent[:, i], noise=n_up)
            out = conv(out, latent[:, i + 1], noise=n_conv)
            skip = to_rgb(out, latent[:, i + 2], skip)
            i += 2
        return (skip, latent) if return_latents else (skip, None)
```

include/gg_b200.h:

```cpp
#ifndef GG_B200_H_
#define GG_B200_H_

#include <stdint.h>

#ifdef __cplusplus
extern "C" {
#endif

#define GG_API __attribute__((visibility("default")))

enum { GG_F32 = 0, GG_F16 = 1, GG_BF16 = 2, GG_F64 = 3 };

enum {
  GG_OK = 0,
  GG_ERR_BAD_ARG = -1,
  GG_ERR_UNSUPPORTED = -2,
  GG_ERR_CUDA = -3
};

enum { GG_PAD_ZEROS = 0, GG_PAD_BORDER = 1, GG_PAD_REFLECTION = 2 };

GG_API int gg_version(void);
GG_API const char* gg_last_error(void);
GG_API int gg_sm_count(void);

GG_API int gg_fused_bias_act(void* out, const void* x, const void* bias, const void* ref, int dtype,
                             int act, int grad, float alpha, float scale, int64_t size_x,
                             int64_t step_b, int64_t size_b, void* stream);

GG_API int gg_noise_bias_act(void* out, const void* x, const void* noise, const float* noise_weight,
                             const float* bias, const float* row_scale, int dtype, float alpha, float scale,
                             int64_t N, int64_t C, int64_t HW, void* stream);

GG_API int64_t gg_channel_scale_workspace(int64_t rows, int64_t HW);
GG_API int gg_channel_scale(void* out, float* row_dot, void* workspace, const void* x, const void* y,
                            const float* s, int dtype, int64_t rows, int64_t HW, void* stream);

GG_API int64_t gg_bias_act_backward_workspace(int64_t N, int64_t C, int64_t HW);
GG_API int gg_bias_act_backward(void* gx, float* grad_bias, void* workspace, const void* g,
                                const void* out, int dtype, float alpha, float scale, int64_t N,
                                int64_t C, int64_t HW, void* stream);

GG_API int gg_upfirdn2d(void* out, const void* in, const float* kernel, int dtype, int64_t major,
                        int in_h, int in_w, int kernel_h, int kernel_w, int up_x, int up_y,
                        int down_x, int down_y, int pad_x0, int pad_x1, int pad_y0, int pad_y1,
                        void* stream);

GG_API int gg_blur_noise_bias_act(void* out, const void* in, const float* kernel, const void* noise,
                                  const float* noise_weight, const float* bias,
                                  const float* row_scale, int dtype, int64_t N, int64_t C, int in_h,
                                  int in_w, int kernel_h, int kernel_w, int pad_x0, int pad_x1,
                                  int pad_y0, int pad_y1, int act, float alpha, float scale,
                                  void* stream);

GG_API int64_t gg_mipmap_pyramid_elems(int64_t planes, int hs, int ws, int extra_levels);
GG_API int gg_mipmap_build(float* pyramid, const void* src, int dtype, int64_t planes, int hs, int ws,
                           int extra_levels, void* stream);
GG_API int gg_mipmap_build_backward(float* grad_src, float* grad_pyramid, int64_t planes, int hs, int ws,
                                    int extra_levels, void* stream);
GG_API int gg_mipmap_warp_forward(void* out, float* levels_out, const void* src, const float* pyramid,
                                  const float* grid, int dtype, int64_t N, int C, int hs, int ws, int ho,
                                  int wo, int extra_levels, float max_level, float min_level,
                                  int padding_mode, void* stream);
GG_API int gg_mipmap_warp_backward(float* grad_src, float* grad_pyramid, float* grad_grid,
                                   const void* grad_out, const void* src, const float* pyramid,
                                   const float* grid, int dtype, int64_t N, int C, int hs, int ws, int ho,
                                   int wo, int extra_levels, float max_level, float min_level,
                                   int padding_mode, void* stream);
GG_API int gg_warp_sample_indices(int32_t* indices, const float* grid, int64_t N, int hs, int ws, int ho, int wo,
                                  float max_level, float min_level, int padding_mode, void* stream);
GG_API int gg_mipmap_warp_lerp_forward(void* out, float* grid_out, const void* src, const float* pyramid, const float* base,
                                       int64_t base_stride, const float* target, const float* alphas, int T, int dtype,
                                       int64_t N, int C, int hs, int ws, int ho, int wo, int extra_levels, float max_level,
                                       float min_level, int padding_mode, void* stream);
GG_API int gg_mipmap_warp_lerp_mean(float* acc, const void* src, const float* pyramid, const float* base, int64_t base_stride,
                                    const float* target, const float* alphas, int T, int dtype, int64_t N, int C, int hs,
                                    int ws, int ho, int wo, int extra_levels, float max_level, float min_level,
                                    int padding_mode, int accumulate, void* stream);

GG_API int gg_flow_compose_forward(float* delta_flow, float* flow, const float* low_flow, const float* mask,
                                   const float* identity_flow, const float* base_warp, const float* alpha,
                                   int64_t N, int H, int W, int S, void* stream);
GG_API int gg_flow_compose_backward(float* grad_mask, float* grad_low_flow, float* grad_base_warp,
                                    const float* grad_delta, const float* grad_flow, const float* low_flow,
                                    const float* mask, const float* identity_flow, const float* base_warp,
                                    const float* alpha, int64_t N, int H, int W, int S, void* stream);

GG_API int64_t gg_splat2d_workspace(int64_t N, int C, int H, int W);
GG_API int gg_splat2d_forward(float* out, void* workspace, const float* input, const float* coordinates,
                              const float* values, const float* sigma, int64_t N, int64_t P, int C, int H,
                              int W, int soft_normalize, void* stream);

GG_API int64_t gg_splat_composite_grid_workspace(int64_t T_chunk, int64_t N, int R, int has_alpha);
GG_API int gg_splat_composite_grid(unsigned char* out, void* workspace, int64_t workspace_bytes, const float* images,
                                   const float* points, const float* colors, const float* alpha, float sigma,
                                   float opacity, int64_t T, int64_t N, int64_t P, int C, int R, int nrow, int padding,
                                   int colors_n, int alpha_n, void* stream);

GG_API int gg_splat_lookup_composite_grid(unsigned char* out, float* points_out, void* workspace, int64_t workspace_bytes,
                                          const float* images, const float* grid, const float* query,
                                          const unsigned char* flip, const float* colors, const float* alpha, float sigma,
                                          float opacity, int64_t N, int64_t P, int query_n, int C, int R, int grid_h,
                                          int grid_w, int nrow, int padding, int colors_n, int alpha_n, void* stream);

GG_API int gg_stn_sample_forward(void* out, float* grid_out, float* delta_out, float* levels_out, const void* src,
                                 const float* pyramid, const float* theta, const float* low, const float* mask,
                                 const float* identity, const float* alpha, int mode, int dtype, int64_t N, int C,
                                 int hs, int ws, int ho, int wo, int lh, int lw, int s, int extra_levels,
                                 float max_level, float min_level, int padding_mode, void* stream);

GG_API int gg_modconv_wsq(float* wsq, const float* weight, int O, int I, int kk, void* stream);
GG_API int gg_modconv_demod(float* demod, const float* wsq, const float* style, float scale, float eps, int B,
                            int O, int I, void* stream);
GG_API int gg_modconv_demod_batched(int layers, float* const* demod, const float* const* wsq, const float* const* style,
                                    const float* scale, const int* O, const int* I, float eps, int B, void* stream);
GG_API int gg_modconv_modulate(float* out, const float* weight, const float* style, const float* demod,
                               float scale, int B, int O, int I, int kk, int transposed, void* stream);

GG_API int gg_noise_bias_act_nhwc(void* out, const void* x, const float* noise, const float* noise_weight,
                                  const float* bias, const float* row_scale, int dtype, float alpha, float scale,
                                  int64_t N, int C, int64_t HW, void* stream);
GG_API int64_t gg_nhwc_rowwise_workspace(int64_t N, int C, int64_t HW);
GG_API int gg_channel_scale_nhwc(void* out, float* row_dot, void* workspace, const void* x, const void* y,
                                 const float* s, int dtype, int64_t N, int C, int64_t HW, void* stream);
GG_API int gg_bias_act_backward_nhwc(void* gx, float* grad_bias, void* workspace, const void* g,
                                     const void* out_saved, int dtype, float alpha, float scale, int64_t N, int C,
                                     int64_t HW, void* stream);
GG_API int64_t gg_blur_nhwc_workspace(int dtype, int64_t N, int C, int in_h, int in_w, int kernel_h, int kernel_w,
                                      int pad_x0, int pad_x1, int pad_y0, int pad_y1);
GG_API int gg_blur_nhwc(void* out, void* out2, const void* in, const float* kernel, const float* noise,
                        const float* noise_weight, const float* bias, const float* row_scale, const float* scale2,
                        const void* mul, float* row_dot, void* workspace, int dtype, int64_t N, int C, int in_h,
                        int in_w, int kernel_h, int kernel_w, int separable, int pad_x0, int pad_x1, int pad_y0,
                        int pad_y1, int mode, int act, float alpha, float scale, void* stream);
GG_API int gg_blur_nhwc_mask(void* mask, void* out2, const void* in, const float* kernel, const float* noise,
                             const float* noise_weight, const float* bias, const float* row_scale, const float* scale2,
                             int dtype, int64_t N, int C, int in_h, int in_w, int kernel_h, int kernel_w, int separable,
                             int pad_x0, int pad_x1, int pad_y0, int pad_y1, int act, float alpha, float scale,
                             void* stream);

GG_API int gg_styled_tail_nhwc(void* out, void* xs, float* rgb, const void* raw, const float* noise,
                               const float* noise_weight, const float* bias, const float* demod, const float* s_next,
                               const float* wm, const float* rgb_bias, const float* skip, int dtype, int act,
                               float alpha, float scale, int64_t N, int C, int64_t HW, void* stream);
GG_API int64_t gg_styled_tail_backward_workspace(int dtype, int64_t N, int C, int64_t HW);
GG_API int gg_styled_tail_backward_nhwc(void* g_raw, float* d_s_next, float* d_demod, float* d_wm, void* workspace,
                                        const void* g_xs, const float* g_rgb, const void* out_saved, const void* raw,
                                        const float* s_next, const float* demod, const float* wm, int dtype,
                                        float alpha, float scale, int64_t N, int C, int64_t HW, int64_t reduce_pitch,
                                        void* stream);
GG_API int gg_styled_tail_mask_nhwc(void* mask, void* xs, float* rgb, const void* raw, const float* noise,
                                    const float* noise_weight, const float* bias, const float* demod,
                                    const float* s_next, const float* wm, const float* rgb_bias, const float* skip,
                                    int dtype, int act, float alpha, float scale, int64_t N, int C, int64_t HW,
                                    void* stream);
GG_API int gg_styled_tail_backward_mask_nhwc(void* g_raw, const void* g_xs, const float* g_rgb, const void* mask,
                                             const float* s_next, const float* demod, const float* wm, int dtype,
                                             float alpha, float scale, int64_t N, int C, int64_t HW, void* stream);

GG_API int64_t gg_to_rgb_nhwc_workspace(int64_t N, int C, int64_t HW);
GG_API int gg_to_rgb_nhwc_forward(float* out, const float* x, const float* wm, const float* bias, const float* skip,
                                  int64_t N, int C, int64_t HW, void* stream);
GG_API int gg_to_rgb_nhwc_backward(float* gx, float* gwm, void* workspace, const float* g, const float* x,
                                   const float* wm, int64_t N, int C, int64_t HW, void* stream);


GG_API int64_t gg_feature_distance_workspace(int64_t N, int C, int64_t HW);
GG_API int gg_feature_distance_forward(float* out, void* workspace, const void* f0, const void* f1,
                                       const float* weight, int dtype, int64_t N, int C, int64_t HW, float eps,
                                       void* stream);
GG_API int gg_feature_distance_backward(void* g0, void* g1, const float* grad_out, const void* f0, const void* f1,
                                        const float* weight, int dtype, int64_t N, int C, int64_t HW, float eps,
                                        void* stream);

GG_API int gg_bias_relu_pool_nhwc_forward(void* y, void* pooled, const void* raw, const float* bias, int dtype, int64_t N,
                                          int C, int H, int W, void* stream);
GG_API int gg_bias_relu_pool_nhwc_backward(void* grad_raw, const void* grad_y, const void* grad_pooled, const void* y,
                                           int dtype, int64_t N, int C, int H, int W, void* stream);

GG_API int gg_tent_downsample_forward(float* out, const float* in, const float* taps_h, const float* taps_v, int64_t N,
                                      int C, int in_h, int in_w, int stride, void* stream);
GG_API int gg_tent_downsample_backward(float* grad_in, const float* grad_out, const float* taps_h, const float* taps_v,
                                       int64_t N, int C, int in_h, int in_w, int stride, void* stream);

GG_API int64_t gg_nn_argmin_workspace(int64_t N, int64_t P);
GG_API int gg_nn_argmin(int64_t* index, void* workspace, const float* grid, const float* points, int64_t N, int64_t P, int HW,
                        void* stream);
GG_API int gg_track_points_lerp(int64_t* track, int64_t* centers, const float* base, const float* target, const float* alphas,
                                const float* points, int T, int64_t N, int64_t P, int H, int W, int patch, void* stream);
GG_API int gg_splat2d_lookup_forward(float* out, float* points_out, void* workspace, const float* input, const float* grid,
                                     const float* query, const float* values, const float* sigma, int64_t N, int64_t P,
                                     int C, int H, int W, int grid_h, int grid_w, float unnorm_k, float unnorm_m,
                                     int soft_normalize, void* stream);

GG_API int gg_tv_per_sample(float* out, const float* flow, int64_t N, int H, int W, void* stream);
GG_API int64_t gg_pck_transfer_workspace(int64_t B, int64_t P, int F);
GG_API int gg_pck_transfer(int64_t* counts, float* est_points, int64_t* nn_index, void* workspace, const float* points,
                           const float* gt_points, const float* visible, const float* thresh, const float* alphas,
                           const float* matrix_src, const float* matrix_dst, const float* delta_src, const float* identity,
                           const float* grid_dst, int64_t B, int64_t P, int A, int S, int F, int grid_h, int grid_w,
                           void* stream);

GG_API int64_t gg_laplacian_blend_workspace(int64_t N, int C, int H, int W, int levels, int backward);
GG_API int gg_laplacian_blend_forward(float* out, void* workspace, const float* img0, const float* img1, const float* mask,
                                      const float* taps, int64_t N, int C, int H, int W, int levels, int width, void* stream);
GG_API int gg_laplacian_blend_backward(float* grad_img0, float* grad_img1, float* grad_mask, void* workspace,
                                       const float* grad_out, const float* img0, const float* img1, const float* mask,
                                       const float* taps, int64_t N, int C, int H, int W, int levels, int width,
                                       void* stream);

GG_API int gg_adam_ema_step(const void* table, const int* block_tensor, const int* block_chunk, int blocks, int chunk,
                            float* state, double beta1, double beta2, double eps, double ema_decay, void* stream);
GG_API int64_t gg_tv_loss_workspace(int64_t N, int H, int W);
GG_API int gg_tv_loss_forward(float* out, void* workspace, const float* flow, int64_t N, int H, int W, void* stream);
GG_API int gg_tv_loss_backward(float* grad_flow, const float* grad_out, const float* flow, int64_t N, int H, int W,
                               void* stream);

GG_API int gg_scale_cast_multi(const void* table, const int* block_tensor, const int* block_chunk, int blocks, int chunk,
                               void* stream);

GG_API int gg_batch_gram(double* gram, double* mean, const float* w, const int64_t* batch_offsets, int64_t B, int D,
                         void* stream);

GG_API int gg_flow_image_grid(unsigned char* out, void* workspace, const float* flow, int64_t N, int H, int W, int nrow,
                              int padding, void* stream);
GG_API int gg_image_grid(unsigned char* out, const float* images, const float* ranges, int64_t N, int H, int W, int nrow,
                         int padding, void* stream);
GG_API int gg_cluster_accumulate(float* sums, int64_t* counts, float* keep, const float* images, const int64_t* sel,
                                 int64_t N, int S, int K, int C, int H, int W, int64_t stride_n, int64_t stride_flip,
                                 int64_t stride_head, int64_t stride_c, int64_t stride_h, int64_t stride_w, int n_keep,
                                 void* stream);

#ifdef __cplusplus
}
#endif
#endif
```

Measured before the change: 494.6.

## Fuse ResBlock bias-act into blur and residual add with sign-mask backward

Adds a blur kernel mode that applies bias and leaky ReLU to each staged input tile before blurring, plus a fused bias-act-plus-skip-add kernel. Both record a packed one-bit-per-element sign mask, which a new mask-driven backward uses in place of re-reading the saved full-precision activation. The discriminator ResBlock forward is rewired to use these paths, removing separate elementwise passes and the residual add. In exchange the blur kernel does extra shared-memory work and a barrier per stage, and the new paths only apply when C is a multiple of 32.

```diff
diff --git a/gangealing_b200/_lib.py b/gangealing_b200/_lib.py
--- a/gangealing_b200/_lib.py
+++ b/gangealing_b200/_lib.py
@@ -44,6 +44,9 @@
     "gg_blur_nhwc_workspace": (_L, [_I, _L] + [_I] * 9),
     "gg_blur_nhwc": (_I, [_P] * 12 + [_I, _L] + [_I] * 12 + [_F, _F, _P]),
     "gg_blur_nhwc_mask": (_I, [_P] * 9 + [_I, _L] + [_I] * 11 + [_F, _F, _P]),
+    "gg_bias_act_blur_nhwc": (_I, [_P] * 5 + [_I, _L] + [_I] * 10 + [_F, _F, _P]),
+    "gg_bias_act_add_nhwc": (_I, [_P] * 5 + [_I, _F, _F, _L, _I, _L, _P]),
+    "gg_bias_act_backward_mask_nhwc": (_I, [_P] * 5 + [_I, _F, _F, _L, _I, _L, _P]),
     "gg_styled_tail_nhwc": (_I, [_P] * 12 + [_I, _I, _F, _F, _L, _I, _L, _P]),
     "gg_styled_tail_mask_nhwc": (_I, [_P] * 12 + [_I, _I, _F, _F, _L, _I, _L, _P]),
     "gg_styled_tail_backward_mask_nhwc": (_I, [_P] * 7 + [_I, _F, _F, _L, _I, _L, _P]),
diff --git a/gangealing_b200/csrc/nhwc.cu b/gangealing_b200/csrc/nhwc.cu
--- a/gangealing_b200/csrc/nhwc.cu
+++ b/gangealing_b200/csrc/nhwc.cu
@@ -59,11 +59,65 @@
   }
 }
 
+template <typename T> __device__ __forceinline__ float stored(float v) { return v; }
+template <> __device__ __forceinline__ float stored<__nv_bfloat16>(float v) {
+  return __bfloat162float(__float2bfloat16_rn(v));
+}
+
+template <typename T>
+__global__ void __launch_bounds__(kT)
+bias_act_add_nhwc_kernel(T* __restrict__ out, uint32_t* __restrict__ mask, const T* __restrict__ x,
+                         const T* __restrict__ skip, const float* __restrict__ bias, float alpha, float gain, int64_t n_vec,
+                         int cv) {
+  constexpr int V = ChanVec<T>::V;
+  const int64_t base = (static_cast<int64_t>(blockIdx.x) * 4) * kT + threadIdx.x;
+  uint4 xv[4], sv[4];
+#pragma unroll
+  for (int u = 0; u < 4; ++u) {
+    const int64_t v = base + static_cast<int64_t>(u) * kT;
+    if (v < n_vec) {
+      xv[u] = ldg_stream16(x + v * V);
+      sv[u] = skip ? ldg_stream16(skip + v * V) : make_uint4(0u, 0u, 0u, 0u);
+    }
+  }
+#pragma unroll
+  for (int u = 0; u < 4; ++u) {
+    const int64_t v = base + static_cast<int64_t>(u) * kT;
+    const bool live = v < n_vec;
+    const int cq = n_vec <= 0xffffffffLL ? static_cast<int>(static_cast<unsigned>(v) % static_cast<unsigned>(cv))
+                                         : static_cast<int>(v % cv);
+    float a[V], o[V];
+#pragma unroll
+    for (int k = 0; k < V; ++k) a[k] = o[k] = 0.f;
+    if (live) {
+      float xf[V], sf[V];
+      ChanVec<T>::unpack(xv[u], xf);
+      ChanVec<T>::unpack(sv[u], sf);
+#pragma unroll
+      for (int q = 0; q < V / 4; ++q) {
+        const float4 b = __ldg(reinterpret_cast<const float4*>(bias) + cq * (V / 4) + q);
+        const float bb[4] = {b.x, b.y, b.z, b.w};
+#pragma unroll
+        for (int k = 0; k < 4; ++k) {
+          const float t = __fadd_rn(__fadd_rn(xf[4 * q + k], bb[k]), 0.f);
+          a[4 * q + k] = stored<T>(__fmul_rn(t > 0.f ? t : __fmul_rn(t, alpha), gain));
+          o[4 * q + k] = skip ? __fadd_rn(a[4 * q + k], sf[4 * q + k]) : a[4 * q + k];
+        }
+      }
+    }
+    const uint32_t word = sign_word<V>(sign_bits<float, V>(a), cq, 0xffffffffu);
+    if (live) {
+      stg_stream16(out + v * V, ChanVec<T>::pack(o));
+      if ((cq * V & 31) == 0) mask[(v * V) >> 5] = word;
+    }
+  }
+}
+
 template <typename T, int MODE>
 __global__ void __launch_bounds__(kT)
 rowwise_nhwc_kernel(T* __restrict__ out, float* __restrict__ partial, const T* __restrict__ x,
-                    const T* __restrict__ y, const float* __restrict__ s, float alpha, float gain, int cv,
-                    int64_t hw, int chunk, int chunks_per_sample) {
+                    const T* __restrict__ y, const uint32_t* __restrict__ mask, const float* __restrict__ s, float alpha,
+                    float gain, int cv, int64_t hw, int chunk, int chunks_per_sample) {
   constexpr int V = ChanVec<T>::V;
   extern __shared__ float red[];
   const int64_t n = blockIdx.x / chunks_per_sample;
@@ -79,8 +133,12 @@
     float sv[V];
 #pragma unroll
     for (int k = 0; k < V; ++k) sv[k] = (MODE == 0) ? __ldg(s + n * cv * V + cq * V + k) : 1.f;
-    const bool has_y = (MODE == 1) || y != nullptr;
-    auto body = [&](const uint4 xr, const uint4 yr, int64_t off) {
+    const bool has_y = (MODE == 1) || (MODE == 0 && y != nullptr);
+    const int words = cv * V / 32;
+    auto bits_at = [&](int64_t pix) -> uint32_t {
+      return MODE == 2 ? sign_load<V>(mask + pix * words, cq) : 0u;
+    };
+    auto body = [&](const uint4 xr, const uint4 yr, uint32_t bits, int64_t off) {
       float xf[V], yf[V], o[V];
       ChanVec<T>::unpack(xr, xf);
       ChanVec<T>::unpack(yr, yf);
@@ -90,7 +148,8 @@
           o[k] = xf[k] * sv[k];
           if (has_y) acc[k] = fmaf(xf[k], yf[k], acc[k]);
         } else {
-          o[k] = (yf[k] > 0.f ? xf[k] : xf[k] * alpha) * gain;
+          const bool pos = MODE == 1 ? yf[k] > 0.f : ((bits >> k) & 1u) != 0u;
+          o[k] = (pos ? xf[k] : xf[k] * alpha) * gain;
           acc[k] += o[k];
         }
       }
@@ -100,6 +159,7 @@
     int64_t p = p0 + pl;
     for (; p + 3 * lanes_p < p1; p += 4 * lanes_p) {
       uint4 xv[4], yv[4];
+      uint32_t bv[4];
       int64_t off[4];
 #pragma unroll
       for (int u = 0; u < 4; ++u) {
@@ -107,15 +167,18 @@
         xv[u] = ldg_stream16(x + off[u]);
       }
 #pragma unroll
-      for (int u = 0; u < 4; ++u) yv[u] = has_y ? ldg_stream16(y + off[u]) : zero;
-#pragma unroll
-      for (int u = 0; u < 4; ++u) body(xv[u], yv[u], off[u]);
+      for (int u = 0; u < 4; ++u) {
+        yv[u] = has_y ? ldg_stream16(y + off[u]) : zero;
+        bv[u] = bits_at(n * hw + p + u * lanes_p);
+      }
+#pragma unroll
+      for (int u = 0; u < 4; ++u) body(xv[u], yv[u], bv[u], off[u]);
     }
     for (; p < p1; p += lanes_p) {
       const int64_t off = ((n * hw + p) * cv + cq) * V;
       const uint4 xv = ldg_stream16(x + off);
       const uint4 yv = has_y ? ldg_stream16(y + off) : zero;
-      body(xv, yv, off);
+      body(xv, yv, bits_at(n * hw + p), off);
     }
   }
   if (partial) {
@@ -294,11 +357,12 @@
                  const float* __restrict__ filt, int kh, int kw, const float* __restrict__ noise,
                  const float* __restrict__ noise_weight, const float* __restrict__ bias,
                  const float* __restrict__ row_scale, const float* __restrict__ scale2, const T* __restrict__ mul,
-                 float* __restrict__ partial, BlurNhwcParams p) {
+                 uint32_t* __restrict__ mask, float* __restrict__ partial, BlurNhwcParams p) {
   using G = BlurGeom<T>;
   constexpr int V = G::V, CB = G::CB, COLS = G::COLS, BX = G::BX, TW = G::TW;
   constexpr bool FUSED = MODE == 1 || MODE == 3;
   constexpr bool MASK = MODE == 3;
+  constexpr bool PRE = MODE == 4;
   extern __shared__ __align__(128) unsigned char tiles_raw[];
   T* tiles = reinterpret_cast<T*>(tiles_raw);
   __shared__ uint64_t full_bar[kNS];
@@ -392,6 +456,11 @@
     }
     nw = noise ? (noise_weight ? __ldg(noise_weight) : 1.f) : 0.f;
   }
+  if (PRE) {
+#pragma unroll
+    for (int k = 0; k < V; ++k) bq[k] = __ldg(bias + c0 + cq * V + k);
+  }
+  const bool last_x = bx == static_cast<int>(gridDim.x) / chunks - 1, last_seg = blockIdx.y == gridDim.y - 1;
   constexpr bool fast = FUSED && FAST;
   const float neg = (p.act == 3) ? p.alpha : 1.f;
   if (fast) {
@@ -474,6 +543,36 @@
       }
     }
     mbar_wait(&full_bar[stage], static_cast<uint32_t>((it / kNS) & 1));
+    if constexpr (PRE) {
+      T* sw = tiles + stage * G::STAGE_ELEMS;
+      constexpr int PIX = kRY * TW;
+#pragma unroll
+      for (int j = 0; j < (PIX + 31) / 32; ++j) {
+        const int pix = xg + 32 * j;
+        const bool live = pix < PIX;
+        const int r = pix / TW, i = pix - r * TW;
+        const int r_in_ = it * kRY + r, iy = iy0 + r_in_, ix = ix0 + i;
+        const bool inside = live && iy >= 0 && iy < p.in_h && ix >= 0 && ix < p.in_w;
+        uint4* vp = reinterpret_cast<uint4*>(sw + pix * CB) + cq;
+        float f[V];
+#pragma unroll
+        for (int k = 0; k < V; ++k) f[k] = 0.f;
+        if (inside) {
+          ChanVec<T>::unpack(*vp, f);
+#pragma unroll
+          for (int k = 0; k < V; ++k) {
+            const float t = __fadd_rn(__fadd_rn(f[k], bq[k]), 0.f);
+            f[k] = __fmul_rn(t > 0.f ? t : __fmul_rn(t, p.alpha), p.gain);
+          }
+        }
+        if (live) *vp = ChanVec<T>::pack(f);
+        const uint32_t word = sign_word<V>(sign_bits<T, V>(f), cq, 0xffffffffu);
+        const bool own = inside && (i < BX || last_x) && (r_in_ < rows_out || (last_seg && r_in_ < rows_in));
+        if (own && (cq * V & 31) == 0)
+          mask[((static_cast<int64_t>(n) * p.in_h + iy) * p.in_w + ix) * (p.c >> 5) + ((c0 + cq * V) >> 5)] = word;
+      }
+      __syncthreads();
+    }
     const T* st = tiles + stage * G::STAGE_ELEMS;
 #pragma unroll
     for (int rr = 0; rr < kRY; ++rr, ++r_in, ocur += row_stride) {
@@ -657,8 +756,9 @@
   return N * k * C * static_cast<int64_t>(sizeof(float));
 }
 
-static int launch_rowwise(int mode, void* out, float* dst, void* workspace, const void* x, const void* y, const float* s,
-                          int dtype, float alpha, float gain, int64_t N, int C, int64_t HW, bool per_sample, void* stream) {
+static int launch_rowwise(int mode, void* out, float* dst, void* workspace, const void* x, const void* y,
+                          const uint32_t* mask, const float* s, int dtype, float alpha, float gain, int64_t N, int C,
+                          int64_t HW, bool per_sample, void* stream) {
   if (N < 0 || C < 0 || HW < 0) return fail(GG_ERR_BAD_ARG, "nhwc rowwise: negative size");
   if (dtype != GG_F32 && dtype != GG_BF16) return fail(GG_ERR_UNSUPPORTED, "nhwc rowwise: dtype %d not supported", dtype);
   if (N * HW * C == 0) {
@@ -688,12 +788,17 @@
   if (mode == 0) {
     GG_DISPATCH_T(dtype, "nhwc rowwise",
                   (rowwise_nhwc_kernel<T_, 0><<<g, kT, smem, st>>>(static_cast<T_*>(out), partial, static_cast<const T_*>(x),
-                                                                 dst ? static_cast<const T_*>(y) : nullptr, s, alpha, gain,
-                                                                 cv, HW, chunk, K)));
+                                                                 dst ? static_cast<const T_*>(y) : nullptr, nullptr, s, alpha,
+                                                                 gain, cv, HW, chunk, K)));
+  } else if (mode == 1) {
+    GG_DISPATCH_T(dtype, "nhwc rowwise",
+                  (rowwise_nhwc_kernel<T_, 1><<<g, kT, smem, st>>>(static_cast<T_*>(out), partial, static_cast<const T_*>(x),
+                                                                 static_cast<const T_*>(y), nullptr, s, alpha, gain, cv, HW,
+                                                                 chunk, K)));
   } else {
     GG_DISPATCH_T(dtype, "nhwc rowwise",
-                  (rowwise_nhwc_kernel<T_, 1><<<g, kT, smem, st>>>(static_cast<T_*>(out), partial, static_cast<const T_*>(x),
-                                                                 static_cast<const T_*>(y), s, alpha, gain, cv, HW, chunk, K)));
+                  (rowwise_nhwc_kernel<T_, 2><<<g, kT, smem, st>>>(static_cast<T_*>(out), partial, static_cast<const T_*>(x),
+                                                                 nullptr, mask, s, alpha, gain, cv, HW, chunk, K)));
   }
   GG_CHECK_LAUNCH("nhwc rowwise launch");
   if (dst) {
@@ -709,13 +814,44 @@
                           int dtype, int64_t N, int C, int64_t HW, void* stream) {
   if (!s) return fail(GG_ERR_BAD_ARG, "channel_scale_nhwc: null scale");
   if (row_dot && !y) return fail(GG_ERR_BAD_ARG, "channel_scale_nhwc: row_dot needs y");
-  return launch_rowwise(0, out, row_dot, workspace, x, y, s, dtype, 0.f, 1.f, N, C, HW, true, stream);
+  return launch_rowwise(0, out, row_dot, workspace, x, y, nullptr, s, dtype, 0.f, 1.f, N, C, HW, true, stream);
 }
 
 int gg_bias_act_backward_nhwc(void* gx, float* grad_bias, void* workspace, const void* g, const void* out_saved,
                               int dtype, float alpha, float scale, int64_t N, int C, int64_t HW, void* stream) {
   if (!out_saved) return fail(GG_ERR_BAD_ARG, "bias_act_backward_nhwc: null saved output");
-  return launch_rowwise(1, gx, grad_bias, workspace, g, out_saved, nullptr, dtype, alpha, scale, N, C, HW, false, stream);
+  return launch_rowwise(1, gx, grad_bias, workspace, g, out_saved, nullptr, nullptr, dtype, alpha, scale, N, C, HW, false,
+                        stream);
+}
+
+int gg_bias_act_backward_mask_nhwc(void* gx, float* grad_bias, void* workspace, const void* g, const void* mask, int dtype,
+                                   float alpha, float scale, int64_t N, int C, int64_t HW, void* stream) {
+  if (!mask) return fail(GG_ERR_BAD_ARG, "bias_act_backward_mask_nhwc: null mask");
+  if (C % 32 != 0) return fail(GG_ERR_UNSUPPORTED, "bias_act_backward_mask_nhwc: C must be a multiple of 32");
+  return launch_rowwise(2, gx, grad_bias, workspace, g, nullptr, static_cast<const uint32_t*>(mask), nullptr, dtype, alpha,
+                        scale, N, C, HW, false, stream);
+}
+
+int gg_bias_act_add_nhwc(void* out, void* mask, const void* x, const void* skip, const float* bias, int dtype, float alpha,
+                         float scale, int64_t N, int C, int64_t HW, void* stream) {
+  if (N < 0 || C < 0 || HW < 0) return fail(GG_ERR_BAD_ARG, "bias_act_add_nhwc: negative size");
+  if (dtype != GG_F32 && dtype != GG_BF16) return fail(GG_ERR_UNSUPPORTED, "bias_act_add_nhwc: dtype %d not supported", dtype);
+  if (C % 32 != 0) return fail(GG_ERR_UNSUPPORTED, "bias_act_add_nhwc: C must be a multiple of 32");
+  const int64_t numel = N * HW * C;
+  if (numel == 0) return GG_OK;
+  if (!out || !mask || !x || !bias) return fail(GG_ERR_BAD_ARG, "bias_act_add_nhwc: null tensor");
+  if (!aligned16(out) || !aligned16(x) || !aligned16(skip) || !aligned16(bias))
+    return fail(GG_ERR_BAD_ARG, "bias_act_add_nhwc: out, x, skip and bias must be 16-byte aligned");
+  const int V = vec_of(dtype);
+  const int64_t n_vec = numel / V;
+  const int64_t grid = (n_vec + 4 * kT - 1) / (4 * kT);
+  if (grid > 0x7fffffffLL) return fail(GG_ERR_BAD_ARG, "bias_act_add_nhwc: tensor too large");
+  GG_DISPATCH_T(dtype, "bias_act_add_nhwc",
+                (bias_act_add_nhwc_kernel<T_><<<static_cast<unsigned>(grid), kT, 0, static_cast<cudaStream_t>(stream)>>>(
+                    static_cast<T_*>(out), static_cast<uint32_t*>(mask), static_cast<const T_*>(x),
+                    static_cast<const T_*>(skip), bias, alpha, scale, n_vec, C / V)));
+  GG_CHECK_LAUNCH("bias_act_add_nhwc launch");
+  return GG_OK;
 }
 
 int64_t gg_to_rgb_nhwc_workspace(int64_t N, int C, int64_t HW) { return 3 * gg_nhwc_rowwise_workspace(N, C, HW); }
@@ -814,9 +950,9 @@
 template <typename T>
 static int launch_blur(void* out, void* out2, const void* in, const float* kernel, const float* noise,
                        const float* noise_weight, const float* bias, const float* row_scale, const float* scale2,
-                       const void* mul, float* row_dot, void* workspace, int64_t N, int C, int in_h, int in_w, int kernel_h,
-                       int kernel_w, int separable, int pad_x0, int pad_x1, int pad_y0, int pad_y1, int mode, int act,
-                       float alpha, float scale, void* stream, int dtype, bool out_is_mask) {
+                       const void* mul, void* mask, float* row_dot, void* workspace, int64_t N, int C, int in_h, int in_w,
+                       int kernel_h, int kernel_w, int separable, int pad_x0, int pad_x1, int pad_y0, int pad_y1, int mode,
+                       int act, float alpha, float scale, void* stream, int dtype, bool out_is_mask) {
   using G = BlurGeom<T>;
   BlurPlan pl;
   int rc = blur_plan(&pl, dtype, N, C, in_h, in_w, kernel_h, kernel_w, pad_x0, pad_x1, pad_y0, pad_y1);
@@ -860,7 +996,7 @@
   static DeviceOnce configured;
   if (configured.needed()) {
     cudaError_t e = cudaSuccess;
-    const void* kernels[12] = {reinterpret_cast<const void*>(blur_nhwc_kernel<T, 0, true>),
+    const void* kernels[14] = {reinterpret_cast<const void*>(blur_nhwc_kernel<T, 0, true>),
                               reinterpret_cast<const void*>(blur_nhwc_kernel<T, 0, false>),
                               reinterpret_cast<const void*>(blur_nhwc_kernel<T, 1, true, false>),
                               reinterpret_cast<const void*>(blur_nhwc_kernel<T, 1, false, false>),
@@ -871,8 +1007,10 @@
                               reinterpret_cast<const void*>(blur_nhwc_kernel<T, 3, true, true>),
                               reinterpret_cast<const void*>(blur_nhwc_kernel<T, 3, false, true>),
                               reinterpret_cast<const void*>(blur_nhwc_kernel<T, 2, true>),
-                              reinterpret_cast<const void*>(blur_nhwc_kernel<T, 2, false>)};
-    for (int i = 0; i < 12 && e == cudaSuccess; ++i)
+                              reinterpret_cast<const void*>(blur_nhwc_kernel<T, 2, false>),
+                              reinterpret_cast<const void*>(blur_nhwc_kernel<T, 4, true>),
+                              reinterpret_cast<const void*>(blur_nhwc_kernel<T, 4, false>)};
+    for (int i = 0; i < 14 && e == cudaSuccess; ++i)
       e = cudaFuncSetAttribute(kernels[i], cudaFuncAttributeMaxDynamicSharedMemorySize, static_cast<int>(smem));
     if (e != cudaSuccess) return cuda_fail(e, "blur_nhwc smem opt-in");
     configured.done();
@@ -883,7 +1021,8 @@
 #define GG_BLUR(M_, S_, F_)                                                                                          \
   blur_nhwc_kernel<T, M_, S_, F_><<<grid, kT, smem, st>>>(static_cast<T*>(out), static_cast<T*>(out2), tmap, kernel, kernel_h, \
                                                          kernel_w, noise, noise_weight, bias, row_scale, scale2,     \
-                                                         static_cast<const T*>(mul), partial, p)
+                                                         static_cast<const T*>(mul), static_cast<uint32_t*>(mask),   \
+                                                         partial, p)
   if (mode == 1 && out_is_mask) {
     if (fast) { if (separable) GG_BLUR(3, true, true); else GG_BLUR(3, false, true); }
     else { if (separable) GG_BLUR(3, true, false); else GG_BLUR(3, false, false); }
@@ -893,6 +1032,7 @@
     else { if (separable) GG_BLUR(1, true, false); else GG_BLUR(1, false, false); }
   }
   else if (mode == 2) { if (separable) GG_BLUR(2, true, false); else GG_BLUR(2, false, false); }
+  else if (mode == 4) { if (separable) GG_BLUR(4, true, false); else GG_BLUR(4, false, false); }
   else { if (separable) GG_BLUR(0, true, false); else GG_BLUR(0, false, false); }
 #undef GG_BLUR
   GG_CHECK_LAUNCH("blur_nhwc launch");
@@ -923,8 +1063,8 @@
   if (N > 65535) return fail(GG_ERR_UNSUPPORTED, "blur_nhwc: batch > 65535");
   if (mode == 0) { noise = nullptr; noise_weight = nullptr; bias = nullptr; row_scale = nullptr; scale2 = nullptr; }
   GG_DISPATCH_T(dtype, "blur_nhwc",
-                return launch_blur<T_>(out, out2, in, kernel, noise, noise_weight, bias, row_scale, scale2, mul, row_dot,
-                                       workspace, N, C, in_h, in_w, kernel_h, kernel_w, separable, pad_x0, pad_x1, pad_y0,
+                return launch_blur<T_>(out, out2, in, kernel, noise, noise_weight, bias, row_scale, scale2, mul, nullptr,
+                                       row_dot, workspace, N, C, in_h, in_w, kernel_h, kernel_w, separable, pad_x0, pad_x1, pad_y0,
                                        pad_y1, mode, act, alpha, scale, stream, dtype, false));
   return GG_OK;
 }
@@ -944,9 +1084,34 @@
   if (N > 65535) return fail(GG_ERR_UNSUPPORTED, "blur_nhwc_mask: batch > 65535");
   GG_DISPATCH_T(dtype, "blur_nhwc_mask",
                 return launch_blur<T_>(mask, out2, in, kernel, noise, noise_weight, bias, row_scale, scale2, nullptr, nullptr,
-                                       nullptr, N, C, in_h, in_w, kernel_h, kernel_w, separable, pad_x0, pad_x1, pad_y0,
+                                       nullptr, nullptr, N, C, in_h, in_w, kernel_h, kernel_w, separable, pad_x0, pad_x1, pad_y0,
                                        pad_y1, 1, act, alpha, scale, stream, dtype, true));
   return GG_OK;
 }
 
-}
+static int trunk_blur_args(const char* who, int64_t N, int C, int in_h, int in_w, int kernel_h, int kernel_w, int dtype) {
+  if (N < 0 || C < 0 || in_h < 1 || in_w < 1) return fail(GG_ERR_BAD_ARG, "%s: bad shape", who);
+  if (kernel_h < 1 || kernel_w < 1 || kernel_h > 4 || kernel_w > 4) return fail(GG_ERR_UNSUPPORTED, "%s: filter must be <= 4x4", who);
+  if (dtype != GG_F32 && dtype != GG_BF16) return fail(GG_ERR_UNSUPPORTED, "%s: dtype %d not supported (fp32 or bf16)", who, dtype);
+  if (C % 32 != 0) return fail(GG_ERR_UNSUPPORTED, "%s: C must be a multiple of 32", who);
+  if (N > 65535) return fail(GG_ERR_UNSUPPORTED, "%s: batch > 65535", who);
+  return GG_OK;
+}
+
+int gg_bias_act_blur_nhwc(void* out, void* mask, const void* in, const float* kernel, const float* bias, int dtype, int64_t N,
+                          int C, int in_h, int in_w, int kernel_h, int kernel_w, int separable, int pad_x0, int pad_x1,
+                          int pad_y0, int pad_y1, float alpha, float scale, void* stream) {
+  int rc = trunk_blur_args("bias_act_blur_nhwc", N, C, in_h, in_w, kernel_h, kernel_w, dtype);
+  if (rc != GG_OK) return rc;
+  if (pad_x0 < 0 || pad_y0 < 0 || pad_x1 < kernel_w - 4 || pad_y1 < kernel_h - 4)
+    return fail(GG_ERR_UNSUPPORTED, "bias_act_blur_nhwc: the blur windows must cover the input (pads >= 0, >= kernel - 4)");
+  if (N == 0 || C == 0) return GG_OK;
+  if (!out || !mask || !in || !kernel || !bias) return fail(GG_ERR_BAD_ARG, "bias_act_blur_nhwc: null tensor");
+  GG_DISPATCH_T(dtype, "bias_act_blur_nhwc",
+                return launch_blur<T_>(out, nullptr, in, kernel, nullptr, nullptr, bias, nullptr, nullptr, nullptr, mask,
+                                       nullptr, nullptr, N, C, in_h, in_w, kernel_h, kernel_w, separable, pad_x0, pad_x1,
+                                       pad_y0, pad_y1, 4, 3, alpha, scale, stream, dtype, false));
+  return GG_OK;
+}
+
+}
diff --git a/gangealing_b200/op/fused_act.py b/gangealing_b200/op/fused_act.py
--- a/gangealing_b200/op/fused_act.py
+++ b/gangealing_b200/op/fused_act.py
@@ -65,8 +65,12 @@
 
 class _FusedLeakyReLUGrad(Function):
     @staticmethod
-    def forward(ctx, grad_output, out, negative_slope, scale, want_bias_grad, bias_dtype=None):
-        gx, grad_bias = bias_act_backward_raw(grad_output, out, negative_slope, scale, want_bias_grad)
+    def forward(ctx, grad_output, out, negative_slope, scale, want_bias_grad, bias_dtype=None, mask=None):
+        if mask is not None and grad_output.shape == out.shape:
+            gx, grad_bias = nhwc.bias_act_backward_mask(nhwc.as_activation(grad_output, out.dtype), mask, negative_slope,
+                                                        scale, want_bias_grad)
+        else:
+            gx, grad_bias = bias_act_backward_raw(grad_output, out, negative_slope, scale, want_bias_grad)
         ctx.save_for_backward(out)
         ctx.cfg = (negative_slope, scale)
         if grad_bias is None:
@@ -81,28 +85,32 @@
         negative_slope, scale = ctx.cfg
         bias = gradgrad_bias if (gradgrad_bias is not None and gradgrad_bias.dim() == 1) else None
         gradgrad_out = fused_bias_act_raw(gradgrad_input, bias, out, 3, 1, negative_slope, scale)
-        return gradgrad_out, None, None, None, None, None
+        return gradgrad_out, None, None, None, None, None, None
 
 
 class FusedLeakyReLUFunction(Function):
     @staticmethod
     def forward(ctx, input, bias, negative_slope, scale):
         _lib.require_cuda(input, bias)
-        if nhwc.elementwise_ok(input) and (bias is None or bias.numel() in (0, input.shape[1])):
+        mask = None
+        if nhwc.bias_act_mask_ok(input) and bias is not None and bias.numel() == input.shape[1]:
+            out, mask = nhwc.bias_act_add(input, None, bias, negative_slope, scale)
+        elif nhwc.elementwise_ok(input) and (bias is None or bias.numel() in (0, input.shape[1])):
             b = bias if (bias is not None and bias.numel() > 0) else None
             out = nhwc.noise_bias_act(input, None, None, b, None, negative_slope, scale)
         else:
             out = fused_bias_act_raw(input, bias, None, 3, 0, negative_slope, scale)
-        ctx.save_for_backward(out)
+        ctx.save_for_backward(out, mask)
         ctx.cfg = (negative_slope, scale, bias.dtype if bias is not None else None)
         return out
 
     @staticmethod
     def backward(ctx, grad_output):
-        (out,) = ctx.saved_tensors
+        out, mask = ctx.saved_tensors
         negative_slope, scale, bias_dtype = ctx.cfg
         want_bias = ctx.needs_input_grad[1]
-        grad_input, grad_bias = _FusedLeakyReLUGrad.apply(grad_output, out, negative_slope, scale, want_bias, bias_dtype)
+        grad_input, grad_bias = _FusedLeakyReLUGrad.apply(grad_output, out, negative_slope, scale, want_bias, bias_dtype,
+                                                          mask)
         return grad_input, (grad_bias if want_bias else None), None, None
 
 
diff --git a/gangealing_b200/op/nhwc.py b/gangealing_b200/op/nhwc.py
--- a/gangealing_b200/op/nhwc.py
+++ b/gangealing_b200/op/nhwc.py
@@ -230,3 +230,67 @@
                                                        negative_slope, gain, n, c, h * w, _lib.stream())
     _lib.check(rc, "gg_styled_tail_backward_mask_nhwc")
     return g_raw
+
+
+def trunk_blur_ok(x, kernel, pad):
+    kh, kw = kernel.shape
+    return (blur_ok(x, kh, kw) and bias_act_mask_ok(x) and pad[0] >= 0 and pad[2] >= 0 and pad[1] >= kw - 4
+            and pad[3] >= kh - 4)
+
+
+def bias_act_blur(x, kernel, pad, bias, negative_slope, gain):
+    n, c, in_h, in_w = x.shape
+    taps = _f32(kernel)
+    kh, kw = taps.shape
+    out_h, out_w = in_h + pad[2] + pad[3] - kh + 1, in_w + pad[0] + pad[1] - kw + 1
+    out = torch.empty((n, c, out_h, out_w), dtype=x.dtype, device=x.device, memory_format=CL)
+    mask = sign_mask_empty(n, c, in_h, in_w, x.device)
+    b = _f32(bias, c)
+    rc = _lib.load().gg_bias_act_blur_nhwc(out.data_ptr(), mask.data_ptr(), x.data_ptr(), taps.data_ptr(), b.data_ptr(),
+                                           _lib.dtype_code(x), n, c, in_h, in_w, kh, kw,
+                                           1 if _lib.filter_is_separable(kernel) else 0, pad[0], pad[1], pad[2], pad[3],
+                                           negative_slope, gain, _lib.stream())
+    _lib.check(rc, "gg_bias_act_blur_nhwc")
+    return out, mask
+
+
+def bias_act_add_ok(x, skip):
+    return (bias_act_mask_ok(x) and skip.shape == x.shape and skip.dtype == x.dtype
+            and skip.is_contiguous(memory_format=CL) and _lib.aligned16(skip))
+
+
+def as_activation(g, dtype):
+    g = g.to(dtype).contiguous(memory_format=CL)
+    return g if _lib.aligned16(g) else g.clone(memory_format=CL)
+
+
+def bias_act_mask_ok(x):
+    return rowwise_ok(x) and x.shape[1] % 32 == 0
+
+
+def bias_act_add(x, skip, bias, negative_slope, gain):
+    n, c, h, w = x.shape
+    out = torch.empty_like(x)
+    mask = sign_mask_empty(n, c, h, w, x.device)
+    b = _f32(bias, c)
+    rc = _lib.load().gg_bias_act_add_nhwc(out.data_ptr(), mask.data_ptr(), x.data_ptr(), _lib.ptr(skip), b.data_ptr(),
+                                          _lib.dtype_code(x), negative_slope, gain, n, c, h * w, _lib.stream())
+    _lib.check(rc, "gg_bias_act_add_nhwc")
+    return out, mask
+
+
+def bias_act_backward_mask(g, mask, negative_slope, gain, want_bias_grad):
+    _activation_like(g, g, "bias_act_backward_mask", "g")
+    n, c, h, w = g.shape
+    if mask.shape != (n, h, w, c // 32):
+        raise RuntimeError("bias_act_backward_mask: mask %s for a (%d, %d, %d, %d) gradient" % (tuple(mask.shape), n, c, h, w))
+    lib = _lib.load()
+    gx = torch.empty_like(g)
+    grad_bias = ws = None
+    if want_bias_grad:
+        grad_bias = torch.empty(c, dtype=torch.float32, device=g.device)
+        ws = torch.empty(max(1, lib.gg_nhwc_rowwise_workspace(n, c, h * w) // 4), dtype=torch.float32, device=g.device)
+    rc = lib.gg_bias_act_backward_mask_nhwc(gx.data_ptr(), _lib.ptr(grad_bias), _lib.ptr(ws), g.data_ptr(), mask.data_ptr(),
+                                            _lib.dtype_code(g), negative_slope, gain, n, c, h * w, _lib.stream())
+    _lib.check(rc, "gg_bias_act_backward_mask_nhwc")
+    return gx, grad_bias
diff --git a/gangealing_b200/op/resblock.py b/gangealing_b200/op/resblock.py
--- /dev/null
+++ b/gangealing_b200/op/resblock.py
@@ -0,0 +1,62 @@
+import torch
+from torch.autograd import Function
+from torch.autograd.function import once_differentiable
+
+from .. import _lib
+from . import nhwc
+from .upfirdn2d import grad_pad
+
+
+class _BiasActBlur(Function):
+    @staticmethod
+    def forward(ctx, raw, bias, kernel, pad, negative_slope, gain):
+        out, mask = nhwc.bias_act_blur(raw, kernel, pad, bias.detach(), negative_slope, gain)
+        ctx.save_for_backward(mask, kernel)
+        ctx.cfg = (pad, negative_slope, gain, raw.shape, raw.dtype, bias.dtype)
+        return out
+
+    @staticmethod
+    @once_differentiable
+    def backward(ctx, g):
+        mask, kernel = ctx.saved_tensors
+        pad, negative_slope, gain, in_shape, dtype, bias_dtype = ctx.cfg
+        g = nhwc.as_activation(g, dtype)
+        kh, kw = kernel.shape
+        gp = grad_pad(in_shape[2], in_shape[3], g.shape[2], g.shape[3], kh, kw, (1, 1), (1, 1), pad)
+        g_a = nhwc.blur(g, _lib.flipped_filter(kernel), gp, mode=0)[0]
+        g_raw, grad_bias = nhwc.bias_act_backward_mask(g_a, mask, negative_slope, gain, ctx.needs_input_grad[1])
+        return g_raw, (grad_bias.to(bias_dtype) if grad_bias is not None else None), None, None, None, None
+
+
+class _BiasActAdd(Function):
+    @staticmethod
+    def forward(ctx, x, skip, bias, negative_slope, gain):
+        out, mask = nhwc.bias_act_add(x, skip, bias.detach(), negative_slope, gain)
+        ctx.save_for_backward(mask)
+        ctx.cfg = (negative_slope, gain, x.dtype, bias.dtype)
+        return out
+
+    @staticmethod
+    @once_differentiable
+    def backward(ctx, g):
+        (mask,) = ctx.saved_tensors
+        negative_slope, gain, dtype, bias_dtype = ctx.cfg
+        gx, grad_bias = nhwc.bias_act_backward_mask(nhwc.as_activation(g, dtype), mask, negative_slope, gain,
+                                                    ctx.needs_input_grad[2])
+        return gx, g, (grad_bias.to(bias_dtype) if grad_bias is not None else None), None, None
+
+
+def bias_act_blur_supported(raw, kernel, pad):
+    return raw.is_cuda and nhwc.trunk_blur_ok(raw, kernel, pad)
+
+
+def bias_act_blur(raw, bias, kernel, pad, negative_slope=0.2, gain=2 ** 0.5):
+    return _BiasActBlur.apply(raw, bias, kernel, tuple(pad), negative_slope, gain)
+
+
+def bias_act_add_supported(x, skip):
+    return x.is_cuda and nhwc.bias_act_add_ok(x, skip)
+
+
+def bias_act_add(x, skip, bias, negative_slope=0.2, gain=2 ** 0.5):
+    return _BiasActAdd.apply(x, skip, bias, negative_slope, gain)
diff --git a/gangealing_b200/opset.py b/gangealing_b200/opset.py
--- a/gangealing_b200/opset.py
+++ b/gangealing_b200/opset.py
@@ -22,6 +22,7 @@
         from .evaluation import ops as _ev
         from .op import pca as _pca
         from .op import grids as _grids
+        from .op import resblock as _rb
         _cached = types.SimpleNamespace(
             name="sm_90a",
             upfirdn2d=_op.upfirdn2d,
@@ -58,5 +59,9 @@
             flow_image_grid=_grids.flow_image_grid,
             image_grid=_grids.image_grid,
             cluster_accumulate=_grids.cluster_accumulate,
+            bias_act_blur=_rb.bias_act_blur,
+            bias_act_blur_supported=_rb.bias_act_blur_supported,
+            bias_act_add=_rb.bias_act_add,
+            bias_act_add_supported=_rb.bias_act_add_supported,
         )
     return _cached
diff --git a/gangealing_b200/stylegan2/networks.py b/gangealing_b200/stylegan2/networks.py
--- a/gangealing_b200/stylegan2/networks.py
+++ b/gangealing_b200/stylegan2/networks.py
@@ -298,18 +298,30 @@
 
     def forward(self, input):
         act, skip_conv = self.conv2[-1], self.skip[-1]
-        if (input.is_cuda and isinstance(act, FusedLeakyReLU) and getattr(act.ops, "name", None) == "sm_90a"
+        ops = act.ops
+        if (input.is_cuda and isinstance(act, FusedLeakyReLU) and getattr(ops, "name", None) == "sm_90a"
                 and isinstance(skip_conv, EqualConv2d) and skip_conv.bias is None):
             inv = 1.0 / math.sqrt(2)
-            main = self.conv1(input)
-            for layer in list(self.conv2)[:-1]:
+            act1, rest = self.conv1[-1], list(self.conv2)[:-1]
+            main = self.conv1[0](input)
+            blur = rest[0] if isinstance(rest[0], Blur) else None
+            pad = (blur.pad[0], blur.pad[1], blur.pad[0], blur.pad[1]) if blur is not None else None
+            if (len(self.conv1) == 2 and isinstance(act1, FusedLeakyReLU) and blur is not None
+                    and ops.bias_act_blur_supported(main, blur.kernel, pad)):
+                main = ops.bias_act_blur(main, act1.bias, blur.kernel, pad, act1.negative_slope, act1.scale)
+                rest = rest[1:]
+            else:
+                main = act1(main)
+            for layer in rest:
                 main = layer(main)
-            bias = act.bias if main.dtype == torch.bfloat16 else act.bias.type(main.dtype)
-            main = act.ops.fused_leaky_relu(main, bias, act.negative_slope, act.scale * inv)
             side = input
             for layer in list(self.skip)[:-1]:
                 side = layer(side)
-            return main + skip_conv(side, gain=inv)
+            side = skip_conv(side, gain=inv)
+            if ops.bias_act_add_supported(main, side):
+                return ops.bias_act_add(main, side, act.bias, act.negative_slope, act.scale * inv)
+            bias = act.bias if main.dtype == torch.bfloat16 else act.bias.type(main.dtype)
+            return ops.fused_leaky_relu(main, bias, act.negative_slope, act.scale * inv) + side
         return (self.conv2(self.conv1(input)) + self.skip(input)) / math.sqrt(2)
 
 
diff --git a/include/gg_b200.h b/include/gg_b200.h
--- a/include/gg_b200.h
+++ b/include/gg_b200.h
@@ -138,6 +138,13 @@
                              int dtype, int64_t N, int C, int in_h, int in_w, int kernel_h, int kernel_w, int separable,
                              int pad_x0, int pad_x1, int pad_y0, int pad_y1, int act, float alpha, float scale,
                              void* stream);
+GG_API int gg_bias_act_blur_nhwc(void* out, void* mask, const void* in, const float* kernel, const float* bias, int dtype,
+                                 int64_t N, int C, int in_h, int in_w, int kernel_h, int kernel_w, int separable, int pad_x0,
+                                 int pad_x1, int pad_y0, int pad_y1, float alpha, float scale, void* stream);
+GG_API int gg_bias_act_add_nhwc(void* out, void* mask, const void* x, const void* skip, const float* bias, int dtype,
+                                float alpha, float scale, int64_t N, int C, int64_t HW, void* stream);
+GG_API int gg_bias_act_backward_mask_nhwc(void* gx, float* grad_bias, void* workspace, const void* g, const void* mask,
+                                          int dtype, float alpha, float scale, int64_t N, int C, int64_t HW, void* stream);
 
 GG_API int gg_styled_tail_nhwc(void* out, void* xs, float* rgb, const void* raw, const float* noise,
                                const float* noise_weight, const float* bias, const float* demod, const float* s_next,
```

New measurement: 500.8, median of 6. 1.01x the previous value.
